# hku-mars/BALM

Hardware: AMD Instinct MI355X
Metric: BA iterations/sec (W poses x F plane features) (higher is better)
Workload: dtype f64

## Files before the change

### balm_amd/capi.py

```python
import ctypes as C
import os

import numpy as np

_HERE = os.path.dirname(os.path.abspath(__file__))
LIB_PATH = os.environ.get("BALM_HIP_LIB") or os.path.join(_HERE, "lib", "libbalm_hip.so")

FORM_LEFT, FORM_RIGHT = 0, 1
OK, ERR_ARG, ERR_HIP, ERR_STATE, ERR_TOO_FEW_PLANES, ERR_NUMERIC = range(6)
ABI_VERSION = 6
FLAG_TIMING = 1
FLAG_LOOPBACK_SHARDS = 2
FLAG_SYRK_INT8 = 4
T_MOMENTS, T_FACTORS, T_SYRK, T_ASSEMBLE, T_SOLVE, T_UPDATE, T_BUILD, T_VOXEL, T_COV, T_COMM, T_UPLOAD, T_COUNT = range(12)
TIMING_NAMES = ["moments", "factors", "syrk", "assemble", "solve", "update", "build", "voxel", "cov", "comm", "upload"]

EXPORTS = ["balm_create", "balm_prewarm", "balm_create_multi", "balm_destroy", "balm_set_features", "balm_set_features_cb", "balm_evaluate", "balm_only_residual",
           "balm_solve_damped", "balm_damping_iter", "balm_build_clusters", "balm_build_clusters_planes", "balm_voxel_defaults", "balm_associate", "balm_associate_scans", "balm_get_features", "balm_get_association", "balm_pose_covariance",
           "balm_window_open", "balm_window_add_scan", "balm_window_add_scan_strided", "balm_window_recut", "balm_window_get_points", "balm_window_features", "balm_window_marginalize", "balm_window_info", "balm_window_close",
           "balm_set_allreduce", "balm_comm_unique_id", "balm_comm_init_rank", "balm_comm_info",
           "balm_get_timing", "balm_get_shard_timing", "balm_get_solve_trace", "balm_chain_macro_plan", "balm_reset_timing", "balm_work_model", "balm_last_error", "balm_version", "balm_abi_version"]


class IterLog(C.Structure):
    _fields_ = [("r1", C.c_double), ("r2", C.c_double), ("u", C.c_double), ("v", C.c_double),
                ("q", C.c_double), ("q1", C.c_double), ("accepted", C.c_int), ("hess_evaluated", C.c_int)]


class LMOpts(C.Structure):
    _fields_ = [("form", C.c_int), ("u0", C.c_double), ("max_iter", C.c_int), ("rel_tol", C.c_double),
                ("min_planes_per_pose", C.c_int), ("force_hess", C.c_int), ("no_stop", C.c_int),
                ("verbose", C.c_int), ("reanchor", C.c_int), ("abs_tol", C.c_double)]


class VoxelOpts(C.Structure):
    _fields_ = [("voxel_size", C.c_double), ("eigen_thr", C.c_float * 3), ("min_ps", C.c_int), ("layer_limit", C.c_int),
                ("min_observers", C.c_int), ("fix_frames", C.c_int), ("max_plane_dist", C.c_double),
                ("max_lambda21", C.c_double), ("max_lambda0", C.c_double), ("want_point_features", C.c_int),
                ("fix_point_limit", C.c_int), ("defer_recut", C.c_int)]


ALLREDUCE_FN = C.CFUNCTYPE(C.c_int, C.c_void_p, C.c_long, C.c_void_p)
FILL_CLUSTERS_FN = C.CFUNCTYPE(None, C.c_void_p, C.c_int, C.c_int, C.POINTER(C.c_double))

_LIB = None


class BalmError(RuntimeError):
    def __init__(self, code, msg):
        super().__init__("balm_hip error %d: %s" % (code, msg))
        self.code = code


def lib():
    global _LIB
    if _LIB is None:
        if not os.path.exists(LIB_PATH):
            raise ImportError("libbalm_hip.so is not built (%s missing): run `python -m balm_amd.build`. "
                              "There is no CPU fallback for the HIP path." % LIB_PATH)
        L = C.CDLL(LIB_PATH)
        abi = getattr(L, "balm_abi_version", None)
        abi = abi() if abi is not None else 0
        if abi != ABI_VERSION:
            raise ImportError("libbalm_hip.so has ABI revision %d, this binding was written for %d: rebuild (python -m balm_amd.build)"
                              % (abi, ABI_VERSION))
        L.balm_create.restype = C.c_void_p
        L.balm_create.argtypes = [C.c_int, C.c_int, C.c_int]
        L.balm_create_multi.restype = C.c_void_p
        L.balm_create_multi.argtypes = [C.c_int, C.c_int, C.c_int, C.c_int]
        L.balm_prewarm.argtypes = [C.c_int]
        L.balm_destroy.restype = None
        L.balm_destroy.argtypes = [C.c_void_p]
        L.balm_set_features.argtypes = [C.c_void_p, C.c_int, C.c_void_p, C.c_void_p, C.c_void_p]
        L.balm_set_features_cb.argtypes = [C.c_void_p, C.c_int, FILL_CLUSTERS_FN, C.c_void_p, C.c_void_p, C.c_void_p]
        L.balm_evaluate.argtypes = [C.c_void_p, C.c_int, C.c_void_p, C.c_int, C.c_int, C.c_void_p, C.c_void_p,
                                    C.POINTER(C.c_double)]
        L.balm_only_residual.argtypes = [C.c_void_p, C.c_void_p, C.POINTER(C.c_double)]
        L.balm_solve_damped.argtypes = [C.c_void_p, C.c_void_p, C.c_void_p, C.c_double, C.c_void_p,
                                        C.POINTER(C.c_double)]
        L.balm_damping_iter.argtypes = [C.c_void_p, C.POINTER(LMOpts), C.c_void_p, C.POINTER(IterLog),
                                        C.POINTER(C.c_int)]
        L.balm_build_clusters.argtypes = [C.c_void_p, C.c_int, C.c_void_p, C.c_void_p, C.c_void_p, C.c_long,
                                          C.c_void_p, C.c_void_p, C.c_void_p]
        L.balm_build_clusters_planes.argtypes = [C.c_void_p, C.c_int, C.c_void_p, C.c_void_p, C.c_size_t, C.c_size_t, C.c_void_p,
                                                 C.c_void_p, C.c_void_p]
        L.balm_associate_scans.argtypes = [C.c_void_p, C.POINTER(VoxelOpts), C.c_int, C.c_void_p, C.c_void_p, C.c_size_t,
                                           C.c_void_p, C.POINTER(C.c_int), C.POINTER(C.c_long)]
        L.balm_window_add_scan_strided.argtypes = [C.c_void_p, C.c_void_p, C.c_long, C.c_size_t, C.c_void_p]
        L.balm_window_open.argtypes = [C.c_void_p, C.POINTER(VoxelOpts)]
        L.balm_window_add_scan.argtypes = [C.c_void_p, C.c_void_p, C.c_long, C.c_void_p]
        L.balm_window_recut.argtypes = [C.c_void_p]
        L.balm_window_get_points.argtypes = [C.c_void_p, C.c_void_p, C.c_void_p, C.c_void_p, C.c_long, C.c_void_p]
        L.balm_window_features.argtypes = [C.c_void_p, C.POINTER(C.c_int)]
        L.balm_window_marginalize.argtypes = [C.c_void_p, C.c_int, C.c_void_p]
        L.balm_window_info.argtypes = [C.c_void_p, C.POINTER(C.c_int), C.POINTER(C.c_long), C.POINTER(C.c_long)]
        L.balm_window_close.argtypes = [C.c_void_p]
        L.balm_associate.argtypes = [C.c_void_p, C.POINTER(VoxelOpts), C.c_void_p, C.c_void_p, C.c_long, C.c_void_p,
                                     C.POINTER(C.c_int), C.POINTER(C.c_long)]
        L.balm_get_features.argtypes = [C.c_void_p, C.c_void_p, C.c_void_p, C.c_void_p]
        L.balm_get_association.argtypes = [C.c_void_p, C.c_void_p, C.c_void_p]
        L.balm_voxel_defaults.restype = None
        L.balm_voxel_defaults.argtypes = [C.POINTER(VoxelOpts)]
        L.balm_pose_covariance.argtypes = [C.c_void_p, C.c_void_p, C.c_void_p, C.c_double, C.c_void_p, C.c_void_p]
        L.balm_set_allreduce.argtypes = [C.c_void_p, ALLREDUCE_FN, C.c_void_p]
        L.balm_comm_unique_id.argtypes = [C.c_void_p]
        L.balm_comm_init_rank.argtypes = [C.c_void_p, C.c_int, C.c_int, C.c_void_p]
        L.balm_comm_info.argtypes = [C.c_void_p, C.c_void_p]
        L.balm_get_timing.argtypes = [C.c_void_p, C.c_void_p, C.c_void_p]
        L.balm_get_shard_timing.argtypes = [C.c_void_p, C.c_int, C.c_void_p, C.c_void_p]
        L.balm_get_solve_trace.argtypes = [C.c_void_p, C.c_void_p, C.c_long, C.c_void_p]
        L.balm_chain_macro_plan.argtypes = [C.c_int, C.c_int, C.c_void_p, C.c_long]
        L.balm_reset_timing.argtypes = [C.c_void_p]
        L.balm_work_model.argtypes = [C.c_void_p, C.c_void_p]
        L.balm_last_error.restype = C.c_char_p
        L.balm_last_error.argtypes = [C.c_void_p]
        L.balm_version.restype = C.c_char_p
        _LIB = L
    return _LIB


def chain_macro_plan(panels, helpers):
    tab = np.empty(helpers * 64, np.int32)
    rc = lib().balm_chain_macro_plan(int(panels), int(helpers), tab.ctypes.data_as(C.c_void_p), tab.size)
    if rc != OK:
        raise BalmError(rc, "balm_chain_macro_plan(%d, %d)" % (panels, helpers))
    tab = tab.reshape(helpers, 64)
    return [[(int(e) & 0xffff, int(e) >> 16) for e in row if e >= 0] for row in tab]


def _p(a):
    return None if a is None else a.ctypes.data_as(C.c_void_p)


def _c(a, dtype=np.float64):
    return None if a is None else np.ascontiguousarray(a, dtype=dtype)


class Context:

    def __init__(self, win_size, device=0, flags=0, n_devices=None):
        self.L = lib()
        self.W = int(win_size)
        self.n = 6 * self.W
        if n_devices is None:
            self.h = self.L.balm_create(self.W, int(device), int(flags))
        else:
            self.h = self.L.balm_create_multi(self.W, int(device), int(n_devices), int(flags))
        if not self.h:
            raise BalmError(ERR_HIP, "balm_create(win_size=%d, device=%d, n_devices=%s) failed (no GPU, bad device, or "
                                     "win_size out of range)" % (win_size, device, n_devices))
        self.F = 0
        self._cb = None

    def close(self):
        if getattr(self, "h", None):
            self.L.balm_destroy(self.h)
            self.h = None

    def __del__(self):
        try:
            self.close()
        except Exception:
            pass

    def _check(self, rc):
        if rc != OK:
            raise BalmError(rc, self.L.balm_last_error(self.h).decode())

    def set_features(self, clusters, fix, coeffs):
        clusters, fix, coeffs = _c(clusters), _c(fix), _c(coeffs)
        F = clusters.shape[0]
        assert clusters.shape == (F, self.W, 10), clusters.shape
        assert coeffs.shape == (F,)
        assert fix is None or fix.shape == (F, 10)
        self._check(self.L.balm_set_features(self.h, F, _p(clusters), _p(fix), _p(coeffs)))
        self.F = F

    def set_features_cb(self, per_feature, fix, coeffs):
        tabs = [_c(t) for t in per_feature]
        F = len(tabs)
        assert all(t.shape == (self.W, 10) for t in tabs)
        fix, coeffs = _c(fix), _c(coeffs)
        row = self.W * 10

        failed = []

        def fill(_user, f0, f1, dst):
            out = np.ctypeslib.as_array(dst, shape=((f1 - f0) * row,))
            try:
                for a in range(f0, f1):
                    out[(a - f0) * row:(a - f0 + 1) * row] = tabs[a].reshape(-1)
            except BaseException as exc:
                out[:] = 0.0
                failed.append(exc)

        cb = FILL_CLUSTERS_FN(fill)
        rc = self.L.balm_set_features_cb(self.h, F, cb, None, _p(fix), _p(coeffs))
        if failed:
            self.F = 0
            raise failed[0]
        self._check(rc)
        self.F = F

    def build_clusters(self, F, xyz, feat_id, pose_id, fix, coeffs, want_clusters=True):
        xyz = _c(xyz, np.float32).reshape(-1, 3)
        feat_id, pose_id = _c(feat_id, np.int32), _c(pose_id, np.int32)
        fix, coeffs = _c(fix), _c(coeffs)
        out = np.zeros((F, self.W, 10)) if want_clusters else None
        self._check(self.L.balm_build_clusters(self.h, F, _p(xyz), _p(feat_id), _p(pose_id), xyz.shape[0],
                                               _p(fix), _p(coeffs), _p(out)))
        self.F = F
        return out

    @staticmethod
    def _containers(arrays):
        keep = [np.ascontiguousarray(a, dtype=np.float32) for a in arrays]
        keep = [a.reshape(-1, 3) if a.ndim == 1 else a for a in keep]
        cols = {a.shape[1] for a in keep}
        assert len(cols) == 1 and min(cols) >= 3, "every container: [n, c] float32 with the same c >= 3"
        ptrs = (C.c_void_p * len(keep))(*[a.ctypes.data if a.shape[0] else None for a in keep])
        cnt = (C.c_long * len(keep))(*[a.shape[0] for a in keep])
        return ptrs, cnt, 4 * cols.pop(), keep

    def build_clusters_planes(self, planes, pose_col, fix, coeffs, want_clusters=True):
        ptrs, cnt, stride, keep = self._containers(planes)
        F = len(keep)
        fix, coeffs = _c(fix), _c(coeffs)
        out = np.zeros((F, self.W, 10)) if want_clusters else None
        self._check(self.L.balm_build_clusters_planes(self.h, F, ptrs, cnt, stride, 4 * int(pose_col), _p(fix), _p(coeffs), _p(out)))
        self.F = F
        return out

    def associate_scans(self, scans, poses, voxel_size=2.0, eigen_thresholds=(1.0 / 16, 1.0 / 16, 1.0 / 9), min_ps=15,
                        want_features=True, layer_limit=2, min_observers=2, fix_frames=0, strict=None, want_points=False):
        ptrs, cnt, stride, keep = self._containers(scans)
        poses = _c(poses)
        assert poses.shape[0] == self.W + fix_frames == len(keep), "one scan and one pose per window slot"
        o = self._voxel_opts(voxel_size, eigen_thresholds, min_ps, layer_limit, min_observers, fix_frames, strict, want_points)
        F, nr = C.c_int(0), C.c_long(0)
        self._check(self.L.balm_associate_scans(self.h, C.byref(o), len(keep), ptrs, cnt, stride, _p(poses), C.byref(F), C.byref(nr)))
        self.F = F.value
        return self.F, nr.value, self._association_result(want_features, fix_frames, want_points, sum(a.shape[0] for a in keep))

    def _voxel_opts(self, voxel_size, eigen_thresholds, min_ps, layer_limit, min_observers, fix_frames, strict, want_points):
        o = VoxelOpts()
        self.L.balm_voxel_defaults(C.byref(o))
        o.voxel_size = voxel_size
        o.eigen_thr = (C.c_float * 3)(*[float(t) for t in eigen_thresholds])
        o.min_ps, o.layer_limit, o.min_observers, o.fix_frames = min_ps, layer_limit, min_observers, fix_frames
        if strict is not None:
            o.max_plane_dist, o.max_lambda21, o.max_lambda0 = strict
        o.want_point_features = int(want_points)
        return o

    def _association_result(self, want_features, fix_frames, want_points, n_pts):
        feats = None
        if want_features and self.F > 0:
            cl, co = np.zeros((self.F, self.W, 10)), np.zeros(self.F)
            layer = np.zeros(self.F, dtype=np.int32)
            self._check(self.L.balm_get_features(self.h, _p(cl), _p(co), _p(layer)))
            feats = (cl, co, layer)
            if fix_frames or want_points:
                fix = np.zeros((self.F, 10))
                pf = np.zeros(n_pts, dtype=np.int32) if want_points else None
                self._check(self.L.balm_get_association(self.h, _p(fix), _p(pf)))
                feats = (cl, co, layer, fix, pf)
        return feats

    def associate(self, xyz, frame_id, poses, voxel_size=2.0, eigen_thresholds=(1.0 / 16, 1.0 / 16, 1.0 / 9),
                  min_ps=15, want_features=True, layer_limit=2, min_observers=2, fix_frames=0, strict=None,
                  want_points=False):
        xyz = _c(xyz, np.float32).reshape(-1, 3)
        frame_id, poses = _c(frame_id, np.int32), _c(poses)
        assert poses.shape[0] == self.W + fix_frames, "poses for the marginalised scans too"
        o = self._voxel_opts(voxel_size, eigen_thresholds, min_ps, layer_limit, min_observers, fix_frames, strict, want_points)
        F, nr = C.c_int(0), C.c_long(0)
        self._check(self.L.balm_associate(self.h, C.byref(o), _p(xyz), _p(frame_id), xyz.shape[0], _p(poses),
                                          C.byref(F), C.byref(nr)))
        self.F = F.value
        return self.F, nr.value, self._association_result(want_features, fix_frames, want_points, xyz.shape[0])
# ... 170 lines not shown
```

### balm_amd/csrc/balm_capi.hip

```cpp
#include <algorithm>
#include <array>
#include <atomic>
#include <chrono>
#include <cmath>
#include <cstdio>
#include <cstdlib>
#include <cstring>

#include "balm_internal.h"

using namespace balm;

#define HIP_TRY(expr)                                                                              \
  do {                                                                                             \
    hipError_t e_ = (expr);                                                                        \
    if (e_ != hipSuccess) {                                                                        \
      ctx->err = std::string(#expr) + ": " + hipGetErrorString(e_);                                \
      return BALM_ERR_HIP;                                                                         \
    }                                                                                              \
  } while (0)

namespace {

#ifdef BALM_COLD_TRACE
// ... 72 lines not shown
void collect_timing(balm_ctx *c) {
  for (auto &sp : c->timer.pending) {
    float ms = 0;
    if (hipEventElapsedTime(&ms, sp.a, sp.b) == hipSuccess) { c->timer.ms[sp.slot] += ms; c->timer.cnt[sp.slot]++; }
    c->timer.pool.push_back(sp.a); c->timer.pool.push_back(sp.b);
  }
  c->timer.pending.clear();
}

template <class T>
int dalloc(balm_ctx *ctx, T **p, size_t count) {
  if (*p) { hipFree(*p); *p = nullptr; }
  if (count == 0) count = 1;
  HIP_TRY(hipMalloc((void **)p, count * sizeof(T)));
  return BALM_OK;
}

template <class T>
int keep(balm_ctx *ctx, T **p, size_t *cap, size_t count) {
  if (*p && *cap >= count) return BALM_OK;
  for (int k = 0; k < balm_ctx::LM_GRAPHS; k++)
    if (ctx->lm_graph[k]) { hipGraphExecDestroy(ctx->lm_graph[k]); ctx->lm_graph[k] = nullptr; ctx->lm_graph_form[k] = -1; }
  int rc = dalloc(ctx, p, count + count / 4);
  *cap = rc ? 0 : count + count / 4;
  return rc;
}

template <class T>
int ensure(balm_ctx *ctx, T **p, size_t *cap, size_t count) {
  if (*p && *cap >= count) return BALM_OK;
  for (int k = 0; k < balm_ctx::LM_GRAPHS; k++)
    if (ctx->lm_graph[k]) { hipGraphExecDestroy(ctx->lm_graph[k]); ctx->lm_graph[k] = nullptr; ctx->lm_graph_form[k] = -1; }
  int rc = dalloc(ctx, p, count);
  if (rc) return rc;
  *cap = count;
  return BALM_OK;
}

int stage_begin(balm_ctx *ctx, size_t total_bytes) {
  total_bytes += 16 * 256;
  ctx->stage_off = 0;
  if (ctx->stage_cap >= total_bytes) return BALM_OK;
  if (ctx->d_stage) { hipStreamSynchronize(ctx->stream); hipFree(ctx->d_stage); ctx->d_stage = nullptr; ctx->stage_cap = 0; }
  const size_t want = total_bytes + total_bytes / 8;
  HIP_TRY(hipMalloc((void **)&ctx->d_stage, want));
  ctx->stage_cap = want;
  return BALM_OK;
}

template <class T>
T *stage_take(balm_ctx *ctx, size_t count) {
  const size_t off = (ctx->stage_off + 255) & ~(size_t)255;
  ctx->stage_off = off + count * sizeof(T);
  return reinterpret_cast<T *>(ctx->d_stage + off);
}

int sync_stream(balm_ctx *ctx) {
  HIP_TRY(hipStreamSynchronize(ctx->stream));
  HIP_TRY(hipGetLastError());
  collect_timing(ctx);
  return BALM_OK;
}

long red_dacc_off(const balm_ctx *c) { return (long)c->ntiles * TILE_ELEMS; }
long red_r_off(const balm_ctx *c) { return red_dacc_off(c) + (long)DACC_MAX * c->W; }

bool has_transport(const balm_ctx *ctx) { return ctx->comm || multi_is_loopback(ctx) || ctx->allreduce; }

int hook_allreduce(balm_ctx *ctx, double *buf, long n) {
  if (ctx->comm) { Span sp(ctx, BALM_T_COMM); return comm_allreduce(ctx, buf, n); }
  if (multi_is_loopback(ctx)) { Span sp(ctx, BALM_T_COMM); return loopback_allreduce(ctx, buf, n); }
  if (!ctx->allreduce) return BALM_OK;
  int rc = sync_stream(ctx);
  if (rc) return rc;
  if (ctx->allreduce((void *)buf, n, ctx->allreduce_user) != 0) {
    ctx->err = "all-reduce hook failed";
    return BALM_ERR_STATE;
  }
  return BALM_OK;
}

int set_damping(balm_ctx *ctx, double u) {
  ctx->u_value = u;
  ctx->u_on_device = false;
  return BALM_OK;
}
int push_damping(balm_ctx *ctx) {
  double *slot = ctx->h_scal + 16 + (ctx->u_ring++ & 63);
  *slot = ctx->u_value;
  HIP_TRY(hipMemcpyAsync(ctx->d_scal + SCAL_U, slot, sizeof(double), hipMemcpyHostToDevice, ctx->stream));
  ctx->u_on_device = true;
  return BALM_OK;
}

static void collect_timing_if_idle(balm_ctx *ctx) {
  if (!ctx->timer.on || ctx->timer.pending.empty()) return;
  if (hipStreamSynchronize(ctx->stream) == hipSuccess) collect_timing(ctx);
}

int wait_scalars(balm_ctx *ctx) {
  volatile double *stamp = ctx->h_scal + SCAL_STAMP;
  const double want = (double)ctx->mail_seq;
  const auto t0 = std::chrono::steady_clock::now();
  for (int spin = 0;; spin++) {
    if (*stamp == want) { std::atomic_thread_fence(std::memory_order_acquire); collect_timing_if_idle(ctx); return BALM_OK; }
    if ((spin & 255) == 255 && std::chrono::steady_clock::now() - t0 > std::chrono::microseconds(300)) break;
  }
  int rc = sync_stream(ctx);
  if (rc) return rc;
  if (*stamp != want) { ctx->err = "balm_damping_iter: the iteration's scalars did not arrive"; return BALM_ERR_HIP; }
  return BALM_OK;
}

void drop_lm_graphs(balm_ctx *ctx) {
  for (int k = 0; k < balm_ctx::LM_GRAPHS; k++) {
    if (ctx->lm_graph[k]) hipGraphExecDestroy(ctx->lm_graph[k]);
    ctx->lm_graph[k] = nullptr; ctx->lm_graph_form[k] = -1;
  }
}

int residual_device(balm_ctx *ctx, const double *d_poses, int f0, int f1, int slot, bool defer_sum = false, bool send_mail = false) {
  if (f1 <= f0) {
    HIP_TRY(hipMemsetAsync(ctx->d_scal + slot, 0, sizeof(double), ctx->stream));
    ctx->nr_tmp = 0;
  } else {
    Span sp(ctx, BALM_T_MOMENTS);
    launch_world_moments(ctx->stream, ctx->d_cl, d_poses, ctx->W, f0, f1, ctx->d_C);
    const EigenMail mail{ctx->d_scal, ctx->d_hscal, send_mail ? (double)++ctx->mail_seq : 0.0, slot};
    ctx->nr_tmp = launch_feature_eigen(ctx->stream, ctx->d_C, ctx->has_fix ? ctx->d_fix : nullptr, ctx->d_coe, f0, f1, ctx->d_feat_tmp,
                                       ctx->d_rpart_tmp, send_mail ? &mail : nullptr);
    if (!defer_sum) launch_sum_scalar(ctx->stream, ctx->d_rpart_tmp, ctx->nr_tmp, ctx->d_scal + slot);
  }
  HIP_TRY(hipGetLastError());
  if (defer_sum) return BALM_OK;
  return hook_allreduce(ctx, ctx->d_scal + slot, 1);
}

bool fuse_trial(const balm_ctx *ctx) {
  const char *e = getenv("BALM_FUSE_TRIAL");
  return ctx->W <= 256 && ctx->F > 0 && e && e[0] == '1';
}

static bool syrk_int8_mode(const balm_ctx *ctx) {
  if (ctx->flags & BALM_FLAG_SYRK_INT8) return true;
  const char *m = getenv("BALM_SYRK");
  return m && !strcmp(m, "int8");
}
static bool syrk_int8_for(const balm_ctx *ctx, long K) {
  if (!syrk_int8_mode(ctx)) return false;
  if (const char *m = getenv("BALM_SYRK_INT8_MIN_COLS")) return K >= atol(m);
  return K >= 12288L && ctx->W >= 96;
}

int prepare_evaluate(balm_ctx *ctx, int form, int nf) {
  if (nf <= 0) return BALM_OK;
  const SyrkPlan plan = plan_syrk(ctx->ntiles, 3L * nf);
  int rc;
  size_t gcols = (size_t)plan.Kpad + 64, parts = (size_t)plan.SG * ctx->ntiles;
  if (ctx->sparse && nf == ctx->F) {
    gcols = (size_t)ctx->sp_nchunks * ctx->sp_nsteps * 4 + 64;
    parts = (size_t)ctx->sp_nitems;
  }
  {
    const double *before = ctx->d_Gt;
    if ((rc = ensure(ctx, &ctx->d_Gt, &ctx->cap_Gt, gcols * ctx->npad))) return rc;
    if (ctx->d_Gt != before) ctx->gt_dirty_cols = ~(size_t)0;
  }
  if ((rc = ensure(ctx, &ctx->d_part, &ctx->cap_part, parts * TILE_ELEMS))) return rc;
  if (syrk_int8_for(ctx, 3L * nf) && !(ctx->sparse && nf == ctx->F)) {
    if ((rc = ensure(ctx, &ctx->d_i8, &ctx->cap_i8, syrk_i8_scratch_bytes(ctx->n, 3L * nf, nullptr)))) return rc;
    if (!ctx->d_rowmax) ctx->rowmax_cur_valid = false;
    if (!ctx->d_rowmax2) ctx->rowmax_trial_valid = false;
    if ((rc = ensure(ctx, &ctx->d_rowmax, &ctx->cap_rowmax, (size_t)ctx->npad + 128))) return rc;
    if ((rc = ensure(ctx, &ctx->d_rowmax2, &ctx->cap_rowmax2, (size_t)ctx->npad + 128))) return rc;
    if ((rc = ensure(ctx, &ctx->d_rowmax_part, &ctx->cap_rowmax_part, (size_t)factors_grid(ctx->W, nf, form) * 6 * ctx->W))) return rc;
    HIP_TRY(prepare_device_syrk_i8());
  }
  if ((rc = ensure(ctx, &ctx->d_dpart, &ctx->cap_dpart, (size_t)factors_grid(ctx->W, nf, form) * DACC_MAX * ctx->W))) return rc;
  if (nf == ctx->F && fuse_trial(ctx)) {
    if (ctx->cap_Gt2 < gcols * ctx->npad || ctx->cap_dpart2 < (size_t)factors_grid(ctx->W, nf, form) * DACC_MAX * ctx->W) ctx->gt_trial_valid = false;
    if ((rc = ensure(ctx, &ctx->d_Gt2, &ctx->cap_Gt2, gcols * ctx->npad))) return rc;
    if ((rc = ensure(ctx, &ctx->d_dpart2, &ctx->cap_dpart2, (size_t)factors_grid(ctx->W, nf, form) * DACC_MAX * ctx->W))) return rc;
  }
  return BALM_OK;
}

int evaluate_device(balm_ctx *ctx, int form, const double *d_poses, int f0, int f1, int slot) {
  const int W = ctx->W, nf = f1 - f0;
  const int dacc = form == 0 ? DACC_LEFT : DACC_RIGHT;
  int rc;
  if (nf <= 0) {
    HIP_TRY(hipMemsetAsync(ctx->d_red, 0, ctx->red_len * sizeof(double), ctx->stream));
    if ((rc = hook_allreduce(ctx, ctx->d_red, (long)ctx->red_len))) return rc;
    Span sp(ctx, BALM_T_ASSEMBLE);
    launch_assemble(ctx->stream, form, ctx->d_red, red_dacc_off(ctx), ctx->d_sub, ctx->ntiles, W, ctx->d_H, ctx->d_g,
                    ctx->d_red + red_r_off(ctx), ctx->d_scal + slot);
    return BALM_OK;
  }
  SyrkPlan plan = plan_syrk(ctx->ntiles, 3L * nf);
  if ((rc = prepare_evaluate(ctx, form, nf))) return rc;
  const int nblk = factors_grid(W, nf, form);
  hipStream_t s = ctx->stream;
  if (!(ctx->feat_cur_valid && f0 == 0 && f1 == ctx->F)) {
    Span sp(ctx, BALM_T_MOMENTS);
    launch_world_moments(s, ctx->d_cl, d_poses, W, f0, f1, ctx->d_C);
    ctx->nr_cur = launch_feature_eigen(s, ctx->d_C, ctx->has_fix ? ctx->d_fix : nullptr, ctx->d_coe, f0, f1, ctx->d_feat, ctx->d_rpart);
    ctx->feat_cur_valid = (f0 == 0 && f1 == ctx->F);
  }
  const int nr = ctx->nr_cur;
  const bool sparse = ctx->sparse && f0 == 0 && f1 == ctx->F;
  const size_t kpad = sparse ? (size_t)ctx->sp_nchunks * ctx->sp_nsteps * 4 : (size_t)plan.Kpad;
  if (!(ctx->gt_cur_valid && ctx->feat_cur_valid && f0 == 0 && f1 == ctx->F)) {
    Span sp(ctx, BALM_T_FACTORS);
    const size_t k0 = (size_t)3 * nf, k1 = kpad + 64;
    if (ctx->gt_dirty_cols == ~(size_t)0) {
      HIP_TRY(hipMemsetAsync(ctx->d_Gt, 0, ctx->cap_Gt * sizeof(double), s));
      ctx->gt_dirty_cols = 0;
    } else if (ctx->gt_dirty_cols > k0) {
      HIP_TRY(hipMemsetAsync(ctx->d_Gt + k0 * ctx->npad, 0, (std::max(ctx->gt_dirty_cols, k1) - k0) * ctx->npad * sizeof(double), s));
    }
    ctx->gt_dirty_cols = k0;
    ctx->rowmax_cur_valid = launch_factors(s, form, ctx->d_cl, d_poses, ctx->d_feat, W, ctx->npad, f0, f1, ctx->d_Gt, ctx->d_dpart, nblk,
                                           sparse ? ctx->d_slot : nullptr, (!sparse && syrk_int8_for(ctx, 3L * nf)) ? ctx->d_rowmax : nullptr, ctx->d_rowmax_part);
    ctx->gt_cur_valid = false;
  }
  HIP_TRY(hipGetLastError());
  const bool int8 = !sparse && syrk_int8_for(ctx, 3L * nf);
  {
    Span sp(ctx, BALM_T_SYRK);
    if (sparse) launch_syrk_sparse(s, ctx->d_Gt, ctx->npad, ctx->d_jobs, ctx->d_items, ctx->d_chunk_ids, ctx->sp_nsteps, ctx->sp_nitems, ctx->d_part);
    else if (int8) {
      if (launch_syrk_i8(s, ctx->d_Gt, ctx->npad, ctx->n, 3L * nf, ctx->d_sub, ctx->ntiles, ctx->d_i8, ctx->d_part,
                         ctx->rowmax_cur_valid ? ctx->d_rowmax : nullptr)) { ctx->err = "INT8 SYRK: unsupported size"; return BALM_ERR_ARG; }
      plan.SG = 1;
    }
    else launch_syrk(s, ctx->d_Gt, ctx->npad, ctx->ntiles, ctx->d_jobs, plan, ctx->d_part);
  }
  {
    Span sp(ctx, BALM_T_ASSEMBLE);
    launch_reduce(s, ctx->d_part, plan.SG, (long)ctx->ntiles * TILE_ELEMS, ctx->d_dpart, nblk, dacc * W,
                  ctx->d_rpart, nr, ctx->d_red, red_dacc_off(ctx), red_r_off(ctx), sparse ? ctx->d_csr : nullptr);
  }
  if ((rc = hook_allreduce(ctx, ctx->d_red, (long)ctx->red_len))) return rc;
  {
    Span sp(ctx, BALM_T_ASSEMBLE);
    launch_assemble(s, form, ctx->d_red, red_dacc_off(ctx), ctx->d_sub, ctx->ntiles, W, ctx->d_H, ctx->d_g, ctx->d_red + red_r_off(ctx),
                    ctx->d_scal + slot);
  }
  return BALM_OK;
}

int trial_device(balm_ctx *ctx, int form, const double *d_poses, int slot) {
  const int W = ctx->W, F = ctx->F;
  hipStream_t s = ctx->stream;
  const SyrkPlan plan = plan_syrk(ctx->ntiles, 3L * F);
  const bool sparse = ctx->sparse;
  const size_t kpad = sparse ? (size_t)ctx->sp_nchunks * ctx->sp_nsteps * 4 : (size_t)plan.Kpad;
  const int nblk = factors_grid(W, F, form);
  {
    Span sp(ctx, BALM_T_FACTORS);
    const size_t k0 = (size_t)3 * F, k1 = kpad + 64;
    HIP_TRY(hipMemsetAsync(ctx->d_Gt2 + k0 * ctx->npad, 0, (k1 - k0) * ctx->npad * sizeof(double), s));
    if (ctx->npad > ctx->n)
      HIP_TRY(hipMemset2DAsync(ctx->d_Gt2 + ctx->n, (size_t)ctx->npad * sizeof(double), 0,
                               (size_t)(ctx->npad - ctx->n) * sizeof(double), k0, s));
    ctx->nr_tmp = launch_moments_factors(s, form, ctx->d_cl, d_poses, ctx->has_fix ? ctx->d_fix : nullptr, ctx->d_coe, W, ctx->npad, F,
                                         ctx->d_Gt2, ctx->d_dpart2, nblk, sparse ? ctx->d_slot : nullptr, ctx->d_feat_tmp, ctx->d_rpart_tmp,
                                         (!sparse && syrk_int8_for(ctx, 3L * F) && ctx->d_rowmax2) ? ctx->d_rowmax2 : nullptr, ctx->d_rowmax_part);
    ctx->rowmax_trial_valid = !sparse && syrk_int8_for(ctx, 3L * F) && ctx->d_rowmax2;
  }
  HIP_TRY(hipGetLastError());
  {
    Span sp(ctx, BALM_T_MOMENTS);
    launch_sum_scalar(s, ctx->d_rpart_tmp, ctx->nr_tmp, ctx->d_scal + slot);
  }
  ctx->gt_trial_valid = true;
  return hook_allreduce(ctx, ctx->d_scal + slot, 1);
}

int read_scalars(balm_ctx *ctx) {
  HIP_TRY(hipMemcpyAsync(ctx->h_scal, ctx->d_scal, 16 * sizeof(double), hipMemcpyDeviceToHost, ctx->stream));
  return sync_stream(ctx);
}

std::vector<unsigned char> obs_of(const double *clusters, int F, int W) {
  std::vector<unsigned char> obs((size_t)F * W);
  parallel_ranges(obs.size(), (size_t)1 << 16, [&](size_t lo, size_t hi) {
    for (size_t t = lo; t < hi; t++) obs[t] = clusters[t * 10 + 9] != 0 ? 1 : 0;
  });
  return obs;
}

int feature_bookkeeping(balm_ctx *ctx, int F, const unsigned char *obs, const double *fix, const double *coeffs) {
  const int W = ctx->W;
  ctx->planes_per_pose.assign(W, 0);
  double S = 0, B = 0;
  int bad_a = F, bad_rc = BALM_OK;
  std::mutex mu;
  parallel_ranges((size_t)F, (size_t)(65536 / W + 1), [&](size_t lo, size_t hi) {
    std::vector<int> ppp((size_t)W, 0);
    double s = 0, b = 0;
    int my_bad = F, my_rc = BALM_OK;
    for (size_t a = lo; a < hi; a++) {
      int na = 0;
      const unsigned char *oa = obs + a * W;
      for (int i = 0; i < W; i++)
        if (oa[i]) { ppp[(size_t)i]++; na++; }
      if (my_rc == BALM_OK) {
        if (na == 0 && !(fix && fix[a * 10 + 9] != 0)) { my_bad = (int)a; my_rc = BALM_ERR_NUMERIC; }
        else if (!(coeffs[a] >= 0) || !std::isfinite(coeffs[a])) { my_bad = (int)a; my_rc = BALM_ERR_ARG; }
      }
      s += na; b += 0.5 * na * (na + 1.0);
    }
    std::lock_guard<std::mutex> lk(mu);
    for (int i = 0; i < W; i++) ctx->planes_per_pose[(size_t)i] += ppp[(size_t)i];
    S += s; B += b;
    if (my_rc != BALM_OK && my_bad < bad_a) { bad_a = my_bad; bad_rc = my_rc; }
  });
  if (bad_rc == BALM_ERR_NUMERIC) {
    ctx->err = "feature " + std::to_string(bad_a) + " has no observation and no fix cluster (zero point count)";
    return BALM_ERR_NUMERIC;
  }
  if (bad_rc == BALM_ERR_ARG) {
    ctx->err = "feature " + std::to_string(bad_a) + " has a negative or non-finite weight";
    return BALM_ERR_ARG;
  }
  ctx->work_S = S; ctx->work_B = B;
  return BALM_OK;
}

}

extern "C" {

const char *balm_version(void) { return "balm_hip 0.6.0 (gfx950)"; }
int balm_abi_version(void) { return BALM_ABI_VERSION; }

const char *balm_last_error(balm_ctx *ctx) { return ctx ? ctx->err.c_str() : "null context"; }

static void one_destroy(balm_ctx *ctx);

balm_ctx *balm_create(int win_size, int device, int flags) {
  if (win_size < 1 || win_size > MAX_W) return nullptr;
  cold_mark("balm_create: enter");
  int ndev = 0;
  if (hipGetDeviceCount(&ndev) != hipSuccess || ndev < 1 || device < 0 || device >= ndev) return nullptr;
  if (hipSetDevice(device) != hipSuccess) return nullptr;
  cold_mark("balm_create: hipGetDeviceCount + hipSetDevice");
  warm_start(device);
  if (prepare_device_accum() != hipSuccess || prepare_device_cov() != hipSuccess) return nullptr;
  cold_mark("balm_create: prepare_device (function attributes -> code objects)");
  balm_ctx *ctx = new balm_ctx();
  ctx->W = win_size;
  ctx->n = 6 * win_size;
  ctx->npad = (ctx->n + TILE - 1) / TILE * TILE;
  ctx->T = ctx->npad / TILE;
  ctx->nA = (ctx->n + NB - 1) / NB * NB;
  ctx->device = device;
  ctx->flags = flags;
  ctx->timer.on = (flags & BALM_FLAG_TIMING) != 0;
  auto fail = [&]() -> balm_ctx * { one_destroy(ctx); return nullptr; };
  std::vector<int> jobs, sub;
  {
    const int T = ctx->T, ngroups = T / 5;
    std::vector<std::array<int, 3>> mixed[4];
    std::vector<std::array<int, 2>> pairs;
    for (int r = 0; r < TM; r++) for (int c = r; c < TM; c++) pairs.push_back({r, c});
    for (int k = 0; k < 15; k++) mixed[1].push_back({0, pairs[k][0], pairs[k][1]});
    for (int k = 0; k < 10; k++) mixed[1].push_back({1, pairs[k][0], pairs[k][1]});
    for (int k = 10; k < 15; k++) mixed[2].push_back({1, pairs[k][0], pairs[k][1]});
    for (int k = 0; k < 15; k++) mixed[2].push_back({2, pairs[k][0], pairs[k][1]});
    for (int k = 0; k < 5; k++) mixed[2].push_back({3, pairs[k][0], pairs[k][1]});
    for (int k = 5; k < 15; k++) mixed[3].push_back({3, pairs[k][0], pairs[k][1]});
    for (int k = 0; k < 15; k++) mixed[3].push_back({4, pairs[k][0], pairs[k][1]});
    auto regular = [&](int I, int J) {
      jobs.insert(jobs.end(), {0, I, J, 0});
      for (int t = 0; t < 25; t++) sub.push_back(((TM * I + t / TM) << 16) | (TM * J + t % TM));
    };
    for (int m = 0; m < T; m++) {
      for (int i = 0; i < m; i++) regular(i, m);
      if (m >= TM * ngroups) regular(m, m);
      else if (m % TM == TM - 1) {
        const int b = m - (TM - 1);
        for (int v = 1; v <= 3; v++) {
          jobs.insert(jobs.end(), {v, b, b, 0});
          for (const auto &e : mixed[v]) sub.push_back(((TM * (b + e[0]) + e[1]) << 16) | (TM * (b + e[0]) + e[2]));
        }
      }
    }
  }
  ctx->ntiles = (int)(jobs.size() / 4);
  ctx->h_jobs = jobs;
  if (hipStreamCreateWithFlags(&ctx->stream, hipStreamNonBlocking) != hipSuccess) return fail();
  cold_mark("balm_create: job tables + stream");
  const int W = ctx->W, n = ctx->n, nA = ctx->nA;
  ctx->red_len = (size_t)ctx->ntiles * TILE_ELEMS + (size_t)DACC_MAX * W + 2;
  if (dalloc(ctx, &ctx->d_poses, (size_t)12 * W) || dalloc(ctx, &ctx->d_poses_tmp, (size_t)12 * W) ||
      dalloc(ctx, &ctx->d_red, ctx->red_len) || dalloc(ctx, &ctx->d_jobs, jobs.size()) || dalloc(ctx, &ctx->d_sub, sub.size()) ||
      dalloc(ctx, &ctx->d_H, (size_t)n * n) || dalloc(ctx, &ctx->d_g, (size_t)n) ||
      dalloc(ctx, &ctx->d_A, (size_t)(2 * nA + NB) * nA) || dalloc(ctx, &ctx->d_Wp, (size_t)2 * NB * (2 * nA + NB)) ||
      dalloc(ctx, &ctx->d_dvec, (size_t)nA) || dalloc(ctx, &ctx->d_z, (size_t)nA) || dalloc(ctx, &ctx->d_x, (size_t)16 * nA) ||
      dalloc(ctx, &ctx->d_perm, (size_t)nA) || dalloc(ctx, &ctx->d_flags, (size_t)2 * (2 * (nA / NB) + 1) * (nA / NB) + (nA / NB) + 8) || dalloc(ctx, &ctx->d_minv, (size_t)2 * (nA / NB) * NB * NB) || dalloc(ctx, &ctx->d_dx, (size_t)n) ||
      dalloc(ctx, &ctx->d_scal, (size_t)16) || dalloc(ctx, &ctx->d_pre, (size_t)W + 2))
    return fail();
  if (hipHostMalloc((void **)&ctx->h_scal, (16 + 64 + 8) * sizeof(double), hipHostMallocMapped | hipHostMallocCoherent) != hipSuccess) return fail();
  if (hipHostGetDevicePointer((void **)&ctx->d_hscal, ctx->h_scal, 0) != hipSuccess) return fail();
  ctx->h_scal[SCAL_STAMP] = 0.0;
  if (hipMemcpy(ctx->d_jobs, jobs.data(), jobs.size() * sizeof(int), hipMemcpyHostToDevice) != hipSuccess ||
      hipMemcpy(ctx->d_sub, sub.data(), sub.size() * sizeof(int), hipMemcpyHostToDevice) != hipSuccess)
    return fail();
  if (getenv("BALM_SOLVE_TRACE")) {
    const size_t cnt = (size_t)(2 * (nA / NB) + 1) * (nA / NB) * 6 + (size_t)(nA / NB) * 6;
    if (hipMalloc((void **)&ctx->d_trace, cnt * sizeof(long long)) != hipSuccess) return fail();
    hipMemset(ctx->d_trace, 0, cnt * sizeof(long long));
  }
  {
    std::vector<int> ident(nA);
    for (int i = 0; i < nA; i++) ident[i] = i;
    if (hipMemcpy(ctx->d_perm, ident.data(), (size_t)nA * sizeof(int), hipMemcpyHostToDevice) != hipSuccess) return fail();
  }
  if (hipMemset(ctx->d_scal, 0, 16 * sizeof(double)) != hipSuccess) return fail();
  if (hipMemset(ctx->d_red, 0, ctx->red_len * sizeof(double)) != hipSuccess) return fail();
  if (hipMemset(ctx->d_minv, 0, (size_t)2 * (nA / NB) * NB * NB * sizeof(double)) != hipSuccess) return fail();
  cold_mark("balm_create: device buffers + small copies");
  context_born(device); ctx->counted_live = true;
  return ctx;
}

static void one_destroy(balm_ctx *ctx) {
  if (!ctx) return;
  if (ctx->counted_live) { context_gone(ctx->device); ctx->counted_live = false; }
  comm_destroy(ctx);
  drop_lm_graphs(ctx);
  hipSetDevice(ctx->device);
  if (ctx->stream) hipStreamSynchronize(ctx->stream);
  if (ctx->window) { window_close(ctx->window); ctx->window = nullptr; }
  void *ptrs[] = {ctx->d_cl, ctx->d_fix, ctx->d_coe, ctx->d_poses, ctx->d_poses_tmp, ctx->d_C, ctx->d_feat,
                  ctx->d_Gt, ctx->d_Gt2, ctx->d_dpart2, ctx->d_part, ctx->d_dpart, ctx->d_rpart, ctx->d_feat_tmp, ctx->d_rpart_tmp, ctx->d_red, ctx->d_jobs, ctx->d_sub, ctx->d_H,
                  ctx->d_g, ctx->d_A, ctx->d_Wp, ctx->d_dvec, ctx->d_z, ctx->d_x, ctx->d_perm, ctx->d_dx, ctx->d_scal, ctx->d_arena, ctx->d_pre, ctx->d_flags, ctx->d_minv, ctx->d_macro_tab, ctx->d_trace, ctx->d_slot, ctx->d_items, ctx->d_csr, ctx->d_chunk_ids, ctx->d_stage, ctx->d_i8, ctx->d_rowmax, ctx->d_rowmax2, ctx->d_rowmax_part};
  for (void *p : ptrs) if (p) hipFree(p);
  if (ctx->h_scal) hipHostFree(ctx->h_scal);
  ctx->ring.release();
  if (ctx->amail.host) hipHostFree((void *)ctx->amail.host);
  if (ctx->amail.scan_state) hipFree(ctx->amail.scan_state);
  for (auto &sp : ctx->timer.pending) { hipEventDestroy(sp.a); hipEventDestroy(sp.b); }
  for (auto e : ctx->timer.pool) hipEventDestroy(e);
  if (ctx->stream) hipStreamDestroy(ctx->stream);
  delete ctx;
}

static int build_sparse_plan(balm_ctx *ctx, int F, const unsigned char *obs) {
  ctx->sparse = false;
  const char *mode = getenv("BALM_SYRK");
  if (mode && !strcmp(mode, "dense")) return BALM_OK;
  if (syrk_int8_for(ctx, 3L * F)) return BALM_OK;
  const int W = ctx->W, T = ctx->T, ntiles = ctx->ntiles;
  if (T > 128 || T <= 2 || F < 64) return BALM_OK;
  struct Key { uint64_t hi, lo; int a; };
  std::vector<Key> keys((size_t)F);
  parallel_ranges((size_t)F, (size_t)(65536 / W + 1), [&](size_t a0, size_t a1) {
    for (size_t a = a0; a < a1; a++) {
      uint64_t hi = 0, lo = 0;
      const unsigned char *oa = obs + a * W;
      for (int i = 0; i < W; i++)
        if (oa[i])
          for (int b = (6 * i) / TILE; b <= (6 * i + 5) / TILE; b++) {
            if (b < 64) hi |= 1ull << (63 - b); else lo |= 1ull << (127 - b);
          }
      keys[a] = {hi, lo, (int)a};
    }
  });
  auto first_of = [&](const Key &k) { for (int b = 0; b < T; b++) if (b < 64 ? (k.hi >> (63 - b)) & 1 : (k.lo >> (127 - b)) & 1) return b; return T; };
  auto last_of = [&](const Key &k) { for (int b = T - 1; b >= 0; b--) if (b < 64 ? (k.hi >> (63 - b)) & 1 : (k.lo >> (127 - b)) & 1) return b; return -1; };
  std::vector<int> fb((size_t)F), lb((size_t)F);
  for (int a = 0; a < F; a++) { fb[(size_t)a] = first_of(keys[(size_t)a]); lb[(size_t)a] = last_of(keys[(size_t)a]); }
  std::sort(keys.begin(), keys.end(), [&](const Key &x, const Key &y) {
    if (fb[(size_t)x.a] != fb[(size_t)y.a]) return fb[(size_t)x.a] < fb[(size_t)y.a];
    if (lb[(size_t)x.a] != lb[(size_t)y.a]) return lb[(size_t)x.a] < lb[(size_t)y.a];
    return x.hi != y.hi ? x.hi > y.hi : (x.lo != y.lo ? x.lo > y.lo : x.a < y.a);
  });
  const int C = 16, nsteps = 3 * C / 4, nchunks = (F + C - 1) / C;
  auto touched = [](const Key &k, int b) { return b < 64 ? (k.hi >> (63 - b)) & 1 : (k.lo >> (127 - b)) & 1; };
  std::vector<int> slot((size_t)F);
  std::vector<std::vector<int>> chunks_of((size_t)ntiles);
  long total = 0;
  for (int c = 0; c < nchunks; c++) {
    Key cm{0, 0, 0};
    for (int k = c * C; k < F && k < (c + 1) * C; k++) { cm.hi |= keys[(size_t)k].hi; cm.lo |= keys[(size_t)k].lo; slot[(size_t)keys[(size_t)k].a] = k; }
    for (int j = 0; j < ntiles; j++) {
      const int type = ctx->h_jobs[(size_t)4 * j], I = ctx->h_jobs[(size_t)4 * j + 1], J = ctx->h_jobs[(size_t)4 * j + 2];
      bool need;
      if (type == 0) need = touched(cm, I) && touched(cm, J);
      else if (type == 1) need = touched(cm, I) || touched(cm, I + 1);
      else if (type == 2) need = touched(cm, I + 1) || touched(cm, I + 2) || touched(cm, I + 3);
      else need = touched(cm, I + 3) || touched(cm, I + 4);
      if (need) { chunks_of[(size_t)j].push_back(c); total++; }
    }
  }
  const double dense_steps = (double)ntiles * ((3.0 * F + 3) / 4), sparse_steps = (double)total * nsteps;
  const bool forced = mode && !strcmp(mode, "sparse");
  if (total == 0 || (!forced && !(sparse_steps < 0.8 * dense_steps))) return BALM_OK;
  long per = total / 2048;
  if (per < 8) per = 8;
  std::vector<int> items, chunk_ids, csr((size_t)ntiles + 1, 0);
  struct Order { int first_chunk, item; };
  std::vector<Order> order;
  int run = 0;
  for (int j = 0; j < ntiles; j++) {
    csr[(size_t)j] = run;
    const std::vector<int> &L = chunks_of[(size_t)j];
    const long pieces = ((long)L.size() + per - 1) / per;
    for (long q = 0; q < pieces; q++) {
      const size_t b = (size_t)((long)L.size() * q / pieces), e = (size_t)((long)L.size() * (q + 1) / pieces);
      order.push_back({L[b], (int)(items.size() / 4)});
      items.insert(items.end(), {j, (int)chunk_ids.size(), (int)(e - b), run++});
      chunk_ids.insert(chunk_ids.end(), L.begin() + (long)b, L.begin() + (long)e);
    }
  }
  csr[(size_t)ntiles] = run;
  std::stable_sort(order.begin(), order.end(), [](const Order &x, const Order &y) { return x.first_chunk < y.first_chunk; });
  std::vector<int> sorted_items;
  sorted_items.reserve(items.size());
  for (const Order &o : order) sorted_items.insert(sorted_items.end(), items.begin() + 4L * o.item, items.begin() + 4L * o.item + 4);
  if (chunk_ids.empty()) chunk_ids.push_back(0);
  int rc;
  if ((rc = keep(ctx, &ctx->d_slot, &ctx->cap_slot, (size_t)F)) || (rc = keep(ctx, &ctx->d_items, &ctx->cap_items, sorted_items.size())) ||
      (rc = keep(ctx, &ctx->d_chunk_ids, &ctx->cap_chunk_ids, chunk_ids.size())) || (rc = keep(ctx, &ctx->d_csr, &ctx->cap_csr, csr.size())))
    return rc;
  HIP_TRY(hipMemcpy(ctx->d_slot, slot.data(), slot.size() * sizeof(int), hipMemcpyHostToDevice));
  HIP_TRY(hipMemcpy(ctx->d_items, sorted_items.data(), sorted_items.size() * sizeof(int), hipMemcpyHostToDevice));
  HIP_TRY(hipMemcpy(ctx->d_chunk_ids, chunk_ids.data(), chunk_ids.size() * sizeof(int), hipMemcpyHostToDevice));
  HIP_TRY(hipMemcpy(ctx->d_csr, csr.data(), csr.size() * sizeof(int), hipMemcpyHostToDevice));
  ctx->sparse = true; ctx->sp_nsteps = nsteps; ctx->sp_nchunks = nchunks; ctx->sp_nitems = run; ctx->sp_steps = sparse_steps;
  return BALM_OK;
}

static int install_feature_buffers(balm_ctx *ctx, int F, const double *fix, const double *coeffs,
                                   hipMemcpyKind kind = hipMemcpyHostToDevice) {
  int rc;
  drop_lm_graphs(ctx);
  ctx->has_fix = fix != nullptr;
  if (fix) {
    if ((rc = keep(ctx, &ctx->d_fix, &ctx->cap_fix, (size_t)F * 10))) return rc;
    HIP_TRY(hipMemcpyAsync(ctx->d_fix, fix, (size_t)F * 10 * sizeof(double), kind, ctx->stream));
  }
  if ((rc = keep(ctx, &ctx->d_coe, &ctx->cap_coe, (size_t)F))) return rc;
  HIP_TRY(hipMemcpyAsync(ctx->d_coe, coeffs, (size_t)F * sizeof(double), kind, ctx->stream));
  if ((rc = keep(ctx, &ctx->d_C, &ctx->cap_C, (size_t)F * 10))) return rc;
  if ((rc = keep(ctx, &ctx->d_feat, &ctx->cap_feat, (size_t)F * FEAT_STRIDE))) return rc;
  if ((rc = keep(ctx, &ctx->d_feat_tmp, &ctx->cap_feat_tmp, (size_t)F * FEAT_STRIDE))) return rc;
  if ((rc = keep(ctx, &ctx->d_rpart, &ctx->cap_rpart, (size_t)(F + 255) / 256 + 1024 + 1))) return rc;
  if ((rc = keep(ctx, &ctx->d_rpart_tmp, &ctx->cap_rpart_tmp, (size_t)(F + 255) / 256 + 1024 + 1))) return rc;
  ctx->feat_cur_valid = false; ctx->gt_cur_valid = false;
  ctx->F = F;
  return BALM_OK;
}

static int assoc_clusters_host(balm_ctx *ctx);

using FillClusters = std::function<void(int, int, double *, unsigned char *)>;

static int one_set_features_fn(balm_ctx *ctx, int F, const FillClusters &fill, const double *fix, const double *coeffs, bool shard_books = false) {
  if (!ctx) return BALM_ERR_ARG;
  if (ctx->multi && F == 0) { ctx->F = 0; ctx->feat_cur_valid = false; ctx->gt_cur_valid = false; ctx->planes_per_pose.clear(); ctx->work_S = ctx->work_B = 0; return BALM_OK; }
  if (F < 1 || !fill || !coeffs) { ctx->err = "balm_set_features: bad argument"; return BALM_ERR_ARG; }
  HIP_TRY(hipSetDevice(ctx->device));
  const int W = ctx->W;
  const size_t count = (size_t)F * W * 10;
  int rc;
  if ((rc = assoc_clusters_host(ctx))) return rc;
  ctx->F = 0;
  adopt_warm_ring(ctx);
  if ((rc = keep(ctx, &ctx->d_cl, &ctx->cap_cl, count))) return rc;
  if ((rc = stage_begin(ctx, count * sizeof(double)))) return rc;
  double *d_aos = stage_take<double>(ctx, count);
  std::vector<unsigned char> obs((size_t)F * W);
  const size_t unit = (size_t)W * 10 * sizeof(double);
  hipError_t e;
  {
    Span sp(ctx, BALM_T_UPLOAD);
    e = staged_upload(ctx->ring, ctx->device, ctx->stream, d_aos, count * sizeof(double), unit, [&](char *dst, size_t off, size_t len) {
      const int f0 = (int)(off / unit), f1 = f0 + (int)(len / unit);
      fill(f0, f1, reinterpret_cast<double *>(dst), obs.data() + (size_t)f0 * W);
    });
  }
  if (e == hipSuccess) launch_transpose_clusters(ctx->stream, d_aos, ctx->d_cl, F, W);
  HIP_TRY(e);
  if ((!ctx->multi || shard_books) && (rc = feature_bookkeeping(ctx, F, obs.data(), fix, coeffs))) { hipStreamSynchronize(ctx->stream); return rc; }
  if ((rc = build_sparse_plan(ctx, F, obs.data()))) { hipStreamSynchronize(ctx->stream); return rc; }
  if ((rc = install_feature_buffers(ctx, F, fix, coeffs))) { hipStreamSynchronize(ctx->stream); return rc; }
  return sync_stream(ctx);
}

static int one_set_features(balm_ctx *ctx, int F, const double *clusters, const double *fix, const double *coeffs) {
  if (ctx && !(ctx->multi && F == 0) && !clusters) { ctx->err = "balm_set_features: bad argument"; return BALM_ERR_ARG; }
  const size_t row = ctx ? (size_t)ctx->W * 10 : 0;
  return one_set_features_fn(ctx, F, [clusters, row](int f0, int f1, double *dst, unsigned char *o) {
    const double *src = clusters + (size_t)f0 * row;
    stream_copy(dst, src, (size_t)(f1 - f0) * row * sizeof(double));
    const size_t cnt = (size_t)(f1 - f0) * (row / 10);
    for (size_t t = 0; t < cnt; t++) o[t] = src[t * 10 + 9] != 0 ? 1 : 0;
  }, fix, coeffs);
}

static int one_build_clusters(balm_ctx *ctx, int F, const float *xyz, const int *feat_id, const int *pose_id, long n_pts,
// ... 251 lines not shown
  if (arc == -3) { ctx->err = "balm_associate: frame_id out of range or non-finite point"; return BALM_ERR_ARG; }
  if (arc) { ctx->err = arc == -2 ? "balm_associate: unsupported size" : "balm_associate: device failure"; return BALM_ERR_HIP; }
  if (n_root_voxels) *n_root_voxels = nroots;
  if (F == 0) return BALM_OK;
  if (rc) return rc;
  *F_out = F;
  return BALM_OK;
}

static int window_rc(balm_ctx *ctx, const char *who, int rc) {
  if (rc == 0) return BALM_OK;
  ctx->err = std::string(who) + (rc == -2 ? ": window full / bad size / scans that no recut has seen" : rc == -3 ? ": non-finite point or beyond 2^20 voxels" : ": device failure");
  if (rc == -1) ctx->window_dead = true;
  return rc == -1 ? BALM_ERR_HIP : BALM_ERR_ARG;
}

static int window_alive(balm_ctx *ctx, const char *who) {
  if (!ctx->window) { ctx->err = std::string(who) + ": no open window"; return BALM_ERR_STATE; }
  if (ctx->window_dead) { ctx->err = std::string(who) + ": an earlier window call failed on the device; re-open the window (balm_window_open)"; return BALM_ERR_STATE; }
  return BALM_OK;
}

static int one_window_open(balm_ctx *ctx, const balm_voxel_opts *opts) {
  if (!ctx) return BALM_ERR_ARG;
  if (!opts || !(opts->voxel_size > 0) || opts->layer_limit < 0 || opts->layer_limit > 2 || opts->min_observers < 0 || opts->fix_frames < 0 ||
      ctx->W + opts->fix_frames > 512 || opts->max_plane_dist < 0 || opts->max_lambda21 < 0 || opts->max_lambda0 < 0 || opts->fix_point_limit < 0) {
    ctx->err = "balm_window_open: bad argument";
    return BALM_ERR_ARG;
  }
  HIP_TRY(hipSetDevice(ctx->device));
  if (ctx->window) { window_close(ctx->window); ctx->window = nullptr; }
  AssocOpts ao{ctx->W, opts->voxel_size, {opts->eigen_thr[0], opts->eigen_thr[1], opts->eigen_thr[2]}, opts->min_ps, opts->layer_limit,
               opts->min_observers, opts->fix_frames, opts->max_plane_dist, opts->max_lambda21, opts->max_lambda0,
               opts->fix_point_limit > 0 ? opts->fix_point_limit : 50, opts->defer_recut != 0};
  ctx->window = window_open(ctx->stream, ao);
  ctx->window_dead = false;
  if (!ctx->window) { ctx->err = "balm_window_open: allocation failed"; return BALM_ERR_HIP; }
  return BALM_OK;
}

static int one_window_add_scan(balm_ctx *ctx, const float *xyz, long n_pts, const double *pose12) {
  if (!ctx) return BALM_ERR_ARG;
  if (int rcw = window_alive(ctx, "balm_window_add_scan")) return rcw;
  if (!xyz || !pose12 || n_pts < 1) { ctx->err = "balm_window_add_scan: bad argument"; return BALM_ERR_ARG; }
  HIP_TRY(hipSetDevice(ctx->device));
  Span sp(ctx, BALM_T_VOXEL);
  return window_rc(ctx, "balm_window_add_scan", window_add_scan(ctx->window, xyz, n_pts, pose12, true));
}

static int one_window_add_scan_strided(balm_ctx *ctx, const void *points, long n_pts, size_t stride, const double *pose12) {
  if (!ctx) return BALM_ERR_ARG;
  if (int rcw = window_alive(ctx, "balm_window_add_scan")) return rcw;
  StridedPoints sp;
  const void *base[1] = {points};
  const long cnt[1] = {n_pts};
  if (!points || !pose12 || n_pts < 1 || !sp.set(1, base, cnt, stride)) { ctx->err = "balm_window_add_scan_strided: bad argument"; return BALM_ERR_ARG; }
  if (stride == 12) return one_window_add_scan(ctx, static_cast<const float *>(points), n_pts, pose12);
  HIP_TRY(hipSetDevice(ctx->device));
  const size_t bytes = (size_t)n_pts * 12;
  if (bytes > PinnedRing::CHUNK) {
    std::vector<float> flat((size_t)n_pts * 3);
    parallel_ranges((size_t)n_pts, (size_t)1 << 15, [&](size_t lo, size_t hi) { sp.gather(reinterpret_cast<char *>(flat.data() + 3 * lo), (long)lo, (long)(hi - lo)); });
    return one_window_add_scan(ctx, flat.data(), n_pts, pose12);
  }
  adopt_warm_ring(ctx);
  HIP_TRY(ctx->ring.init(ctx->device));
  PinnedRing &ring = ctx->ring;
  const int b = ring.pos;
  if (ring.busy[b]) { HIP_TRY(hipEventSynchronize(ring.ev[b])); ring.busy[b] = false; }
  char *dst = ring.buf[b];
  parallel_ranges((size_t)n_pts, (size_t)1 << 15, [&](size_t lo, size_t hi) {
    sp.gather(dst + 12 * lo, (long)lo, (long)(hi - lo));
  });
  Span span(ctx, BALM_T_VOXEL);
  return window_rc(ctx, "balm_window_add_scan", window_add_scan(ctx->window, reinterpret_cast<const float *>(dst), n_pts, pose12, true));
}

static int one_window_recut(balm_ctx *ctx) {
  if (!ctx) return BALM_ERR_ARG;
  if (int rcw = window_alive(ctx, "balm_window_recut")) return rcw;
  HIP_TRY(hipSetDevice(ctx->device));
  Span sp(ctx, BALM_T_VOXEL);
  return window_rc(ctx, "balm_window_recut", window_recut(ctx->window));
}

static int one_window_marginalize(balm_ctx *ctx, int mg, const double *poses) {
  if (!ctx) return BALM_ERR_ARG;
  if (int rcw = window_alive(ctx, "balm_window_marginalize")) return rcw;
  HIP_TRY(hipSetDevice(ctx->device));
  Span sp(ctx, BALM_T_VOXEL);
  return window_rc(ctx, "balm_window_marginalize", window_marginalize(ctx->window, mg, poses));
}

static int one_window_features(balm_ctx *ctx, int *F_out) {
  if (!ctx) return BALM_ERR_ARG;
  if (int rcw = window_alive(ctx, "balm_window_features")) return rcw;
  if (!F_out) { ctx->err = "balm_window_features: bad argument"; return BALM_ERR_ARG; }
  HIP_TRY(hipSetDevice(ctx->device));
  *F_out = 0;
  ctx->F = 0;
  ctx->assoc_clusters.clear(); ctx->assoc_coeffs.clear(); ctx->assoc_layer.clear(); ctx->assoc_fix.clear(); ctx->assoc_point_feat.clear(); ctx->assoc_cl_on_device = false;
  int F = 0, *d_lay = nullptr;
  double *d_out = nullptr, *d_coe = nullptr, *d_fix = nullptr;
  int rc;
  {
    Span sp(ctx, BALM_T_VOXEL);
    rc = window_features(ctx->window, window_min_observers(ctx->window), &F, &d_out, &d_coe, &d_fix, &d_lay);
  }
  if (rc) return window_rc(ctx, "balm_window_features", rc);
  if (F == 0) return BALM_OK;
  if ((rc = install_associated(ctx, F, d_out, d_coe, d_fix, d_lay, nullptr, 0, true, false))) return rc;
  *F_out = F;
  return BALM_OK;
}

int balm_get_features(balm_ctx *ctx, double *clusters, double *coeffs, int *layer) {
  if (!ctx) return BALM_ERR_ARG;
  if (ctx->assoc_coeffs.empty()) { ctx->err = "balm_get_features: no balm_associate result"; return BALM_ERR_STATE; }
  if (clusters) {
    if (int rc = assoc_clusters_host(ctx)) return rc;
    if (ctx->assoc_clusters.empty()) { ctx->err = "balm_get_features: the association's table is gone"; return BALM_ERR_STATE; }
    std::memcpy(clusters, ctx->assoc_clusters.data(), ctx->assoc_clusters.size() * sizeof(double));
  }
  if (coeffs) std::memcpy(coeffs, ctx->assoc_coeffs.data(), ctx->assoc_coeffs.size() * sizeof(double));
  if (layer) std::memcpy(layer, ctx->assoc_layer.data(), ctx->assoc_layer.size() * sizeof(int));
  return BALM_OK;
}

int balm_get_association(balm_ctx *ctx, double *fix, int *point_feature) {
  if (!ctx) return BALM_ERR_ARG;
  if (ctx->assoc_coeffs.empty()) { ctx->err = "balm_get_association: no balm_associate result"; return BALM_ERR_STATE; }
  if (point_feature && ctx->assoc_point_feat.empty()) {
    ctx->err = "balm_get_association: want_point_features was not set"; return BALM_ERR_STATE;
  }
  if (fix) std::memcpy(fix, ctx->assoc_fix.data(), ctx->assoc_fix.size() * sizeof(double));
  if (point_feature) std::memcpy(point_feature, ctx->assoc_point_feat.data(), ctx->assoc_point_feat.size() * sizeof(int));
  return BALM_OK;
}

static int one_pose_covariance(balm_ctx *ctx, const double *poses, const double *cluster_cov, double point_sigma, double *Rcov,
                         double *Rcov_raw) {
  if (!ctx) return BALM_ERR_ARG;
  if (!ctx->multi && ctx->F < 1) { ctx->err = "balm_pose_covariance: no features installed"; return BALM_ERR_STATE; }
  if (!poses || (!cluster_cov && !(point_sigma > 0))) { ctx->err = "balm_pose_covariance: bad argument"; return BALM_ERR_ARG; }
  if (ctx->W > MAX_W_LDS) { ctx->err = "balm_pose_covariance: windows above 480 poses are not supported"; return BALM_ERR_ARG; }
  HIP_TRY(hipSetDevice(ctx->device));
  const int W = ctx->W, n = ctx->n, nA = ctx->nA, F = ctx->F;
  hipStream_t s = ctx->stream;
  HIP_TRY(hipMemcpyAsync(ctx->d_poses, poses, (size_t)12 * W * sizeof(double), hipMemcpyHostToDevice, s));
  ctx->feat_cur_valid = false; ctx->gt_cur_valid = false;
  int rc = evaluate_device(ctx, BALM_FORM_LEFT, ctx->d_poses, 0, F, 0);
  ctx->feat_cur_valid = false; ctx->gt_cur_valid = false;
  if (rc) return rc;
  const SyrkPlan plan = plan_syrk(ctx->ntiles, 3L * (F > 0 ? F : 1));
  const size_t gcols = (size_t)plan.Kpad + 64, tiles = (size_t)ctx->ntiles * TILE_ELEMS;
  if ((rc = ensure(ctx, &ctx->d_Gt, &ctx->cap_Gt, 2 * gcols * ctx->npad))) return rc;
  ctx->gt_dirty_cols = ~(size_t)0;
  if ((rc = ensure(ctx, &ctx->d_part, &ctx->cap_part, (size_t)plan.SG * tiles))) return rc;
  const int nblk = cov_factors_grid(W, F > 0 ? F : 1);
  if ((rc = ensure(ctx, &ctx->d_dpart, &ctx->cap_dpart, (size_t)nblk * DACC_MAX * W))) return rc;
  const bool int8 = F > 0 && syrk_int8_for(ctx, 3L * F);
  if (int8) {
    if ((rc = ensure(ctx, &ctx->d_i8, &ctx->cap_i8, syrk_i8_scratch_bytes(ctx->n, 3L * F, nullptr)))) return rc;
    HIP_TRY(prepare_device_syrk_i8());
  }
  const size_t pay = 2 * tiles + (size_t)21 * W, nn = (size_t)n * n;
  const size_t ncc = (cluster_cov && F > 0) ? (size_t)F * W * 81 : 0;
  if ((rc = stage_begin(ctx, (pay + 2 * nn + 2 * (size_t)nA * nA + ncc) * sizeof(double)))) return rc;
  double *buf = stage_take<double>(ctx, pay + 2 * nn + 2 * (size_t)nA * nA), *d_cc = nullptr;
  double *redx = buf, *redy = buf + tiles, *sdiag = buf + 2 * tiles, *Rraw = buf + pay, *Rc = Rraw + nn,
         *T0 = Rc + nn, *T1 = T0 + (size_t)nA * nA;
  hipError_t e = hipSuccess;
  if (ncc) {
    d_cc = stage_take<double>(ctx, ncc);
    adopt_warm_ring(ctx);
    if (e == hipSuccess) { Span sp(ctx, BALM_T_UPLOAD); e = staged_copy(ctx->ring, ctx->device, s, d_cc, cluster_cov, (size_t)F * W * 81 * sizeof(double)); }
  }
  double *Gx = ctx->d_Gt, *Gy = ctx->d_Gt + gcols * ctx->npad;
  if (e == hipSuccess && F == 0) e = hipMemsetAsync(buf, 0, pay * sizeof(double), s);
  if (e == hipSuccess && F > 0) {
    Span sp(ctx, BALM_T_COV);
    const size_t k0 = (size_t)3 * F;
    hipMemsetAsync(Gx + k0 * ctx->npad, 0, (gcols - k0) * ctx->npad * sizeof(double), s);
    hipMemsetAsync(Gy + k0 * ctx->npad, 0, (gcols - k0) * ctx->npad * sizeof(double), s);
    launch_cov_factors(s, ctx->d_cl, d_cc, point_sigma * point_sigma, ctx->d_poses, ctx->d_feat, W, ctx->npad, F, Gx, Gy,
                       ctx->d_dpart, nblk);
    e = hipGetLastError();
    if (int8) {
      if (launch_syrk_i8(s, Gx, ctx->npad, ctx->n, 3L * F, ctx->d_sub, ctx->ntiles, ctx->d_i8, ctx->d_part)) e = hipErrorInvalidValue;
      launch_cov_reduce_tiles(s, ctx->d_part, 1, (long)tiles, redx);
      if (launch_syrk_i8(s, Gy, ctx->npad, ctx->n, 3L * F, ctx->d_sub, ctx->ntiles, ctx->d_i8, ctx->d_part)) e = hipErrorInvalidValue;
      launch_cov_reduce_tiles(s, ctx->d_part, 1, (long)tiles, redy);
    } else {
      launch_syrk(s, Gx, ctx->npad, ctx->ntiles, ctx->d_jobs, plan, ctx->d_part);
      launch_cov_reduce_tiles(s, ctx->d_part, plan.SG, (long)tiles, redx);
      launch_syrk(s, Gy, ctx->npad, ctx->ntiles, ctx->d_jobs, plan, ctx->d_part);
      launch_cov_reduce_tiles(s, ctx->d_part, plan.SG, (long)tiles, redy);
    }
    launch_cov_reduce_dacc(s, ctx->d_dpart, nblk, W, sdiag);
  }
  if (e == hipSuccess) rc = hook_allreduce(ctx, buf, (long)pay);
  if (e == hipSuccess && !rc) {
    Span sp(ctx, BALM_T_COV);
    launch_cov_assemble(s, redx, redy, sdiag, ctx->d_sub, ctx->ntiles, W, Rraw);
    hipMemsetAsync(ctx->d_g, 0, (size_t)n * sizeof(double), s);
    set_damping(ctx, 0.0);
    ctx->need_minv = true;
    launch_solve(ctx, true);
    ctx->need_minv = false;
    launch_congruence_inverse(ctx, Rraw, T0, T1, Rc);
    if (Rcov) e = hipMemcpyAsync(Rcov, Rc, nn * sizeof(double), hipMemcpyDeviceToHost, s);
    if (e == hipSuccess && Rcov_raw) e = hipMemcpyAsync(Rcov_raw, Rraw, nn * sizeof(double), hipMemcpyDeviceToHost, s);
  }
  if (e == hipSuccess) e = hipStreamSynchronize(s);
  if (e == hipSuccess) e = hipGetLastError();
  if (rc) return rc;
  HIP_TRY(e);
  collect_timing(ctx);
  return BALM_OK;
}

int balm_comm_info(balm_ctx *ctx, long *out4) {
  if (!ctx || !out4) return BALM_ERR_ARG;
  out4[0] = 1; out4[1] = 0; out4[2] = (long)ctx->red_len; out4[3] = 0;
  if (ctx->comm) {
    int cnt = -1, rk = -1;
    comm_query(ctx, &cnt, &rk);
    out4[0] = cnt; out4[1] = rk; out4[3] = 1;
  } else if (multi_is_loopback(ctx)) {
    out4[0] = ctx->multi->n; out4[1] = ctx->rank; out4[3] = 2;
  } else if (ctx->allreduce) {
    out4[0] = -1; out4[3] = 3;
  }
  return BALM_OK;
}

int balm_set_allreduce(balm_ctx *ctx, balm_allreduce_fn fn, void *user) {
  if (!ctx) return BALM_ERR_ARG;
  if (fn && (ctx->multi || ctx->comm)) { ctx->err = "balm_set_allreduce: the context already has a collective transport"; return BALM_ERR_STATE; }
  ctx->allreduce = fn;
  ctx->allreduce_user = user;
  return BALM_OK;
}

static int one_evaluate(balm_ctx *ctx, int form, const double *poses, int head, int end, double *Hess, double *JacT,
                  double *residual) {
  if (!ctx) return BALM_ERR_ARG;
  if (!ctx->multi) {
    if (ctx->F < 1) { ctx->err = "balm_evaluate: no features installed"; return BALM_ERR_STATE; }
    if ((form != 0 && form != 1) || !poses || head < 0 || end > ctx->F || head >= end) {
      ctx->err = "balm_evaluate: bad argument"; return BALM_ERR_ARG;
    }
  }
  HIP_TRY(hipSetDevice(ctx->device));
  const int n = ctx->n;
  HIP_TRY(hipMemcpyAsync(ctx->d_poses, poses, (size_t)12 * ctx->W * sizeof(double), hipMemcpyHostToDevice, ctx->stream));
  ctx->feat_cur_valid = false; ctx->gt_cur_valid = false;
  int rc = evaluate_device(ctx, form, ctx->d_poses, head, end, 0);
  ctx->feat_cur_valid = false; ctx->gt_cur_valid = false;
  if (rc) return rc;
  if (Hess) HIP_TRY(hipMemcpyAsync(Hess, ctx->d_H, (size_t)n * n * sizeof(double), hipMemcpyDeviceToHost, ctx->stream));
  if (JacT) HIP_TRY(hipMemcpyAsync(JacT, ctx->d_g, (size_t)n * sizeof(double), hipMemcpyDeviceToHost, ctx->stream));
  if ((rc = read_scalars(ctx))) return rc;
  if (residual) *residual = ctx->h_scal[0];
  if (!std::isfinite(ctx->h_scal[0])) { ctx->err = "balm_evaluate: non-finite residual"; return BALM_ERR_NUMERIC; }
  return BALM_OK;
}

static int one_only_residual(balm_ctx *ctx, const double *poses, double *residual) {
  if (!ctx) return BALM_ERR_ARG;
  if (!ctx->multi && ctx->F < 1) { ctx->err = "balm_only_residual: no features installed"; return BALM_ERR_STATE; }
  if (!poses || !residual) { ctx->err = "balm_only_residual: bad argument"; return BALM_ERR_ARG; }
  HIP_TRY(hipSetDevice(ctx->device));
  HIP_TRY(hipMemcpyAsync(ctx->d_poses_tmp, poses, (size_t)12 * ctx->W * sizeof(double), hipMemcpyHostToDevice, ctx->stream));
  int rc = residual_device(ctx, ctx->d_poses_tmp, 0, ctx->F, 1);
  if (rc) return rc;
  if ((rc = read_scalars(ctx))) return rc;
  *residual = ctx->h_scal[1];
  if (!std::isfinite(ctx->h_scal[1])) { ctx->err = "balm_only_residual: non-finite residual"; return BALM_ERR_NUMERIC; }
  return BALM_OK;
}

int balm_solve_damped(balm_ctx *ctx, const double *Hess, const double *JacT, double u, double *dxi, double *q1) {
  if (!ctx) return BALM_ERR_ARG;
  if (!Hess || !JacT || !dxi) { ctx->err = "balm_solve_damped: bad argument"; return BALM_ERR_ARG; }
  HIP_TRY(hipSetDevice(ctx->device));
  const int n = ctx->n;
  HIP_TRY(hipMemcpyAsync(ctx->d_H, Hess, (size_t)n * n * sizeof(double), hipMemcpyHostToDevice, ctx->stream));
  HIP_TRY(hipMemcpyAsync(ctx->d_g, JacT, (size_t)n * sizeof(double), hipMemcpyHostToDevice, ctx->stream));
  {
    Span sp(ctx, BALM_T_SOLVE);
    int rcu = set_damping(ctx, u);
    if (rcu) return rcu;
    launch_solve(ctx, true);
  }
  HIP_TRY(hipMemcpyAsync(dxi, ctx->d_dx, (size_t)n * sizeof(double), hipMemcpyDeviceToHost, ctx->stream));
  int rc = read_scalars(ctx);
  if (rc) return rc;
  if (!std::isfinite(ctx->h_scal[2]) && !ctx->persistent_off && solve_timed_out(ctx)) {
    ctx->persistent_off = true;
    {
      Span sp(ctx, BALM_T_SOLVE);
      launch_solve(ctx, true);
    }
    HIP_TRY(hipMemcpyAsync(dxi, ctx->d_dx, (size_t)n * sizeof(double), hipMemcpyDeviceToHost, ctx->stream));
    if ((rc = read_scalars(ctx))) return rc;
  }
  if (q1) *q1 = ctx->h_scal[2];
  return BALM_OK;
}

static int lm_enqueue(balm_ctx *ctx, int form, bool evaluated, bool mail) {
  int rc;
  if (evaluated && (rc = evaluate_device(ctx, form, ctx->d_poses, 0, ctx->F, 0))) return rc;
  {
    Span sp(ctx, BALM_T_SOLVE);
    launch_solve(ctx, evaluated, form, ctx->d_poses, ctx->d_poses_tmp);
  }
  ctx->gt_trial_valid = false;
  bool sum_in_mail = false;
  if (fuse_trial(ctx) && ctx->d_Gt2 && ctx->d_dpart2) {
    if ((rc = trial_device(ctx, form, ctx->d_poses_tmp, 1))) return rc;
  } else {
    sum_in_mail = mail && !has_transport(ctx) && ctx->F > 0;
    const bool eigen_mails = sum_in_mail && ctx->F <= 256;
    if ((rc = residual_device(ctx, ctx->d_poses_tmp, 0, ctx->F, 1, sum_in_mail, eigen_mails))) return rc;
    if (eigen_mails) return BALM_OK;
  }
  if (mail) launch_scalars_mail(ctx->stream, ctx->d_scal, ctx->d_hscal, (double)++ctx->mail_seq, sum_in_mail ? ctx->d_rpart_tmp : nullptr,
                                ctx->nr_tmp, 1);
  else HIP_TRY(hipMemcpyAsync(ctx->h_scal, ctx->d_scal, 16 * sizeof(double), hipMemcpyDeviceToHost, ctx->stream));
  return BALM_OK;
}

static int lm_iteration(balm_ctx *ctx, int form, bool evaluated, int it) {
  const char *genv = getenv("BALM_GRAPH");
  const bool disabled = !(genv && (!strcmp(genv, "1") || !strcmp(genv, "debug")));
  const bool graphable = !disabled && ctx->graphs_ok && it >= 1 && !ctx->timer.on && !has_transport(ctx) && !ctx->multi &&
                         ctx->feat_cur_valid && ctx->F > 0 && !solve_is_persistent(ctx);
  if (graphable) {
    const bool fused = fuse_trial(ctx) && ctx->d_Gt2 && ctx->d_dpart2;
    const int slot = (ctx->gt_parity ? 16 : 0) | (fused ? 8 : 0) | (ctx->gt_cur_valid ? 4 : 0) | (evaluated ? 2 : 0) | ctx->parity;
    if (ctx->lm_graph[slot] && ctx->lm_graph_form[slot] != form) {
      hipGraphExecDestroy(ctx->lm_graph[slot]); ctx->lm_graph[slot] = nullptr;
    }
    if (!ctx->lm_graph[slot]) {
      hipGraph_t g = nullptr;
      ctx->u_on_device = true;
      bool ok = hipStreamBeginCapture(ctx->stream, hipStreamCaptureModeThreadLocal) == hipSuccess;
      if (ok) {
// ... 382 lines not shown
  for (int a = 0; a < F; a++) cum[(size_t)a + 1] = cum[(size_t)a] + (double)plane_count[a] + 1.0;
  multi_cut(m, F, cum);
  const size_t Wc = (size_t)ctx->W;
  int rc = multi_run(m, [&](int k) {
    const int f0 = m->fbeg[(size_t)k], nf = m->fbeg[(size_t)k + 1] - f0;
    if (nf == 0) return one_set_features(m->sub[(size_t)k], 0, nullptr, nullptr, nullptr);
    StridedPoints part;
    if (!part.set(nf, plane_points + f0, plane_count + f0, stride_bytes, pose_offset_bytes)) return (int)BALM_ERR_ARG;
    return one_build_clusters(m->sub[(size_t)k], nf, nullptr, nullptr, nullptr, 0, fix ? fix + (size_t)f0 * 10 : nullptr, coeffs + f0,
                              clusters_out ? clusters_out + (size_t)f0 * Wc * 10 : nullptr, &part);
  });
  return multi_done(ctx, m, F, rc, "balm_build_clusters_planes");
}

int balm_window_add_scan_strided(balm_ctx *ctx, const void *points, long n_pts, size_t stride_bytes, const double *pose12) {
  return one_window_add_scan_strided(ctx, points, n_pts, stride_bytes, pose12);
}

int balm_window_open(balm_ctx *ctx, const balm_voxel_opts *opts) { return one_window_open(ctx, opts); }
int balm_window_add_scan(balm_ctx *ctx, const float *xyz, long n_pts, const double *pose12) {
  return one_window_add_scan(ctx, xyz, n_pts, pose12);
}
int balm_window_recut(balm_ctx *ctx) { return one_window_recut(ctx); }
int balm_window_marginalize(balm_ctx *ctx, int mg_size, const double *poses) { return one_window_marginalize(ctx, mg_size, poses); }
int balm_window_features(balm_ctx *ctx, int *F_out) {
  balm_multi *m = leader_of(ctx);
  if (!m) return one_window_features(ctx, F_out);
  ctx->multi = nullptr;
  int rc = one_window_features(ctx, F_out);
  ctx->multi = m;
  m->F = 0;
  if (rc || *F_out == 0) return rc;
  if ((rc = assoc_clusters_host(ctx))) return rc;
  return multi_set_features(ctx, m, *F_out, ctx->assoc_clusters.data(), ctx->assoc_fix.data(), ctx->assoc_coeffs.data());
}
int balm_window_info(balm_ctx *ctx, int *scans, long *points, long *nodes) {
  if (!ctx) return BALM_ERR_ARG;
  if (!ctx->window) { ctx->err = "balm_window_info: no open window"; return BALM_ERR_STATE; }
  if (scans) *scans = window_count(ctx->window);
  if (points) *points = window_points(ctx->window);
  if (nodes) *nodes = window_nodes(ctx->window);
  return BALM_OK;
}
int balm_window_get_points(balm_ctx *ctx, float *xyz, int *slot, int *feature, long capacity, long *n_out) {
  if (!ctx) return BALM_ERR_ARG;
  if (int rcw = window_alive(ctx, "balm_window_get_points")) return rcw;
  if (!n_out || capacity < 0) { ctx->err = "balm_window_get_points: bad argument"; return BALM_ERR_ARG; }
  HIP_TRY(hipSetDevice(ctx->device));
  const long n = window_get_points(ctx->window, xyz, slot, feature, capacity);
  if (n == -2) { ctx->err = "balm_window_get_points: capacity too small"; return BALM_ERR_ARG; }
  if (n < 0) return window_rc(ctx, "balm_window_get_points", -1);
  *n_out = n;
  return BALM_OK;
}
int balm_window_close(balm_ctx *ctx) {
  if (!ctx) return BALM_ERR_ARG;
  if (ctx->window) { hipSetDevice(ctx->device); window_close(ctx->window); ctx->window = nullptr; }
  return BALM_OK;
}

int balm_evaluate(balm_ctx *ctx, int form, const double *poses, int head, int end, double *Hess, double *JacT, double *residual) {
  balm_multi *m = leader_of(ctx);
  if (!m) return one_evaluate(ctx, form, poses, head, end, Hess, JacT, residual);
  if (m->F < 1) { ctx->err = "balm_evaluate: no features installed"; return BALM_ERR_STATE; }
  if ((form != 0 && form != 1) || !poses || head < 0 || end > m->F || head >= end) { ctx->err = "balm_evaluate: bad argument"; return BALM_ERR_ARG; }
  return multi_run(m, [&](int k) {
    const int f0 = m->fbeg[(size_t)k], f1 = m->fbeg[(size_t)k + 1];
    const int lh = (head > f0 ? head : f0) - f0, le = (end < f1 ? end : f1) - f0;
    double r = 0;
    return one_evaluate(m->sub[(size_t)k], form, poses, lh, le > lh ? le : lh, k ? nullptr : Hess, k ? nullptr : JacT, k ? &r : residual);
  });
}

int balm_only_residual(balm_ctx *ctx, const double *poses, double *residual) {
  balm_multi *m = leader_of(ctx);
  if (!m) return one_only_residual(ctx, poses, residual);
  if (m->F < 1) { ctx->err = "balm_only_residual: no features installed"; return BALM_ERR_STATE; }
  if (!poses || !residual) { ctx->err = "balm_only_residual: bad argument"; return BALM_ERR_ARG; }
  return multi_run(m, [&](int k) { double r = 0; return one_only_residual(m->sub[(size_t)k], poses, k ? &r : residual); });
}

int balm_damping_iter(balm_ctx *ctx, const balm_lm_opts *o, double *poses, balm_iter_log *log, int *n_iters) {
  balm_multi *m = leader_of(ctx);
  if (!m) return one_damping_iter(ctx, o, poses, log, n_iters);
  if (m->F < 1) { ctx->err = "balm_damping_iter: no features installed"; return BALM_ERR_STATE; }
  if (!o || !poses || o->max_iter < 1) { ctx->err = "balm_damping_iter: bad argument"; return BALM_ERR_ARG; }
  const size_t np = (size_t)12 * ctx->W;
  std::vector<std::vector<double>> pk((size_t)m->n, std::vector<double>(poses, poses + np));
  std::vector<int> its((size_t)m->n, 0);
  balm_lm_opts ok = *o;
  int rc = multi_run(m, [&](int k) {
    balm_lm_opts oo = ok;
    if (k) oo.verbose = 0;
    return one_damping_iter(m->sub[(size_t)k], &oo, pk[(size_t)k].data(), k ? nullptr : log, &its[(size_t)k]);
  });
  if (rc) { if (ctx->err.empty()) for (auto *q : m->sub) if (!q->err.empty()) { ctx->err = q->err; break; } return rc; }
  std::memcpy(poses, pk[0].data(), np * sizeof(double));
  if (n_iters) *n_iters = its[0];
  return BALM_OK;
}

int balm_pose_covariance(balm_ctx *ctx, const double *poses, const double *cluster_cov, double point_sigma, double *Rcov,
                         double *Rcov_raw) {
  balm_multi *m = leader_of(ctx);
  if (!m) return one_pose_covariance(ctx, poses, cluster_cov, point_sigma, Rcov, Rcov_raw);
  if (m->F < 1) { ctx->err = "balm_pose_covariance: no features installed"; return BALM_ERR_STATE; }
  const size_t W = (size_t)ctx->W;
  return multi_run(m, [&](int k) {
    const size_t f0 = (size_t)m->fbeg[(size_t)k];
    return one_pose_covariance(m->sub[(size_t)k], poses, cluster_cov ? cluster_cov + f0 * W * 81 : nullptr, point_sigma,
                               k ? nullptr : Rcov, k ? nullptr : Rcov_raw);
  });
}

int balm_get_solve_trace(balm_ctx *ctx, long long *ticks, long capacity, int *dims3) {
  if (!ctx || !dims3) return BALM_ERR_ARG;
  const int P = ctx->nA / NB, RB = 2 * P + 1;
  dims3[0] = RB; dims3[1] = P; dims3[2] = 6;
  if (!ctx->d_trace) { ctx->err = "balm_get_solve_trace: create the context with BALM_SOLVE_TRACE=1 in the environment"; return BALM_ERR_STATE; }
  if (!ticks || capacity < (long)RB * P * 6 + 6L * P) { ctx->err = "balm_get_solve_trace: buffer too small"; return BALM_ERR_ARG; }
  HIP_TRY(hipSetDevice(ctx->device));
  HIP_TRY(hipStreamSynchronize(ctx->stream));
  HIP_TRY(hipMemcpy(ticks, ctx->d_trace, ((size_t)RB * P * 6 + 6 * (size_t)P) * sizeof(long long), hipMemcpyDeviceToHost));
  return BALM_OK;
}

int balm_get_timing(balm_ctx *ctx, double *ms, long *count) {
  if (!ctx) return BALM_ERR_ARG;
  for (int k = 0; k < BALM_T_COUNT; k++) {
    if (ms) ms[k] = ctx->timer.ms[k];
    if (count) count[k] = ctx->timer.cnt[k];
  }
  return BALM_OK;
}

int balm_get_shard_timing(balm_ctx *ctx, int shard, double *ms, long *count) {
  if (!ctx) return BALM_ERR_ARG;
  balm_ctx *q = ctx;
  if (ctx->multi) {
    if (shard < 0 || shard >= ctx->multi->n) { ctx->err = "balm_get_shard_timing: no such shard"; return BALM_ERR_ARG; }
    q = ctx->multi->sub[(size_t)shard];
  } else if (shard != 0) { ctx->err = "balm_get_shard_timing: no such shard"; return BALM_ERR_ARG; }
  return balm_get_timing(q, ms, count);
}

int balm_chain_macro_plan(int panels, int helpers, int *table, long capacity) {
  if (!table || panels < 3 || helpers < 1 || capacity < (long)helpers * 64) return BALM_ERR_ARG;
  std::vector<int> tab;
  if (!balm::chain_macro_plan(panels, helpers, tab)) return BALM_ERR_ARG;
  memcpy(table, tab.data(), tab.size() * sizeof(int));
  return BALM_OK;
}

int balm_reset_timing(balm_ctx *ctx) {
  if (!ctx) return BALM_ERR_ARG;
  for (int k = 0; k < BALM_T_COUNT; k++) { ctx->timer.ms[k] = 0; ctx->timer.cnt[k] = 0; }
  if (balm_multi *m = leader_of(ctx))
    for (size_t q = 1; q < m->sub.size(); q++)
      for (int k = 0; k < BALM_T_COUNT; k++) { m->sub[q]->timer.ms[k] = 0; m->sub[q]->timer.cnt[k] = 0; }
  return BALM_OK;
}

int balm_work_model(balm_ctx *ctx, double *out4) {
  if (!ctx || !out4) return BALM_ERR_ARG;
  const double W = ctx->W, F = ctx->multi ? ctx->multi->F : ctx->F;
  out4[0] = ctx->work_S;
  out4[1] = ctx->work_B;
  if (ctx->multi && ctx->multi->books_per_shard) {
    out4[0] = out4[1] = 0;
    for (const balm_ctx *q : ctx->multi->sub) { out4[0] += q->work_S; out4[1] += q->work_B; }
  }
  (void)W;
  out4[2] = 216.0 * out4[1];
  SyrkPlan p = plan_syrk(ctx->ntiles, 3L * (long)F);
  out4[3] = (double)ctx->ntiles * 25.0 * 2048.0 * ((double)p.Kpad / 4.0);
  if (ctx->sparse && !ctx->multi) out4[3] = ctx->sp_steps * 25.0 * 2048.0;
  if (ctx->multi) {
    double issued = 0;
    for (size_t k = 0; k < ctx->multi->sub.size(); k++) {
      const balm_ctx *q = ctx->multi->sub[k];
      if (q->F < 1) continue;
      if (q->sparse) issued += q->sp_steps * 25.0 * 2048.0;
      else { const SyrkPlan pk = plan_syrk(q->ntiles, 3L * q->F); issued += (double)q->ntiles * 25.0 * 2048.0 * ((double)pk.Kpad / 4.0); }
    }
    out4[3] = issued;
  }
  return BALM_OK;
}

}
```

### balm_amd/csrc/balm_internal.h

```cpp
#pragma once
#include <hip/hip_runtime.h>
#include <atomic>
#include <condition_variable>
#include <cstddef>
#include <cstdint>
#include <functional>
#include <mutex>
#include <string>
#include <thread>
#include <vector>

#include "../../include/balm_hip.h"
#include "host_stage.h"

namespace balm {

constexpr int TILE = 80;
constexpr int TM = 5;
constexpr int TILE_ELEMS = TILE * TILE;
constexpr int FEAT_STRIDE = 24;
constexpr int DACC_LEFT = 27;
constexpr int DACC_RIGHT = 30;
constexpr int DACC_MAX = 30;
constexpr int NB = 48;
constexpr int MAX_W_LDS = 480;
constexpr int MAX_W = 1024;
constexpr int MAX_SHARDS = 16;

enum { FT_NN = 0, FT_VBAR = 1, FT_LAM = 4, FT_U0 = 7, FT_U1 = 10, FT_U2 = 13, FT_C0 = 16, FT_C1 = 17,
       FT_C2 = 18, FT_COE = 19 };

struct Timer {
  bool on = false;
  struct Span { hipEvent_t a, b; int slot; };
  std::vector<Span> pending;
  std::vector<hipEvent_t> pool;
  double ms[BALM_T_COUNT] = {0};
  long cnt[BALM_T_COUNT] = {0};
};

}

namespace balm {
struct WindowSession;
struct AssocMail {
  volatile unsigned int *host = nullptr; unsigned int *dev = nullptr; unsigned int seq = 0;
  unsigned long long *scan_state = nullptr; unsigned int scan_gen = 0;
};
constexpr long SCAN_TILES_CAP = 8192;
}

struct balm_ctx {
  int W = 0, n = 0, npad = 0, T = 0, ntiles = 0, device = 0, flags = 0;
  int nA = 0;
  int F = 0;
  hipStream_t stream = nullptr;
  std::string err;

  double *d_cl = nullptr;
  double *d_fix = nullptr;
  double *d_coe = nullptr;
  double *d_poses = nullptr;
  double *d_poses_tmp = nullptr;
  double *d_C = nullptr;
  double *d_feat = nullptr;
  double *d_feat_tmp = nullptr;
  double *d_rpart_tmp = nullptr;
  int nr_cur = 0, nr_tmp = 0;
  bool feat_cur_valid = false;
  double *d_Gt = nullptr;
  double *d_Gt2 = nullptr, *d_dpart2 = nullptr;
  size_t cap_Gt2 = 0, cap_dpart2 = 0;
  size_t gt_dirty_cols = ~(size_t)0;
  bool gt_cur_valid = false;
  int gt_parity = 0;
  bool gt_trial_valid = false;
  size_t cap_cl = 0, cap_fix = 0, cap_coe = 0, cap_C = 0, cap_feat = 0, cap_feat_tmp = 0, cap_rpart = 0, cap_rpart_tmp = 0;
  size_t cap_slot = 0, cap_items = 0, cap_chunk_ids = 0, cap_csr = 0;
  bool has_fix = false;
  size_t cap_Gt = 0;
  double *d_part = nullptr;
  size_t cap_part = 0;
  double *d_dpart = nullptr;
  size_t cap_dpart = 0;
  double *d_rpart = nullptr;
  double *d_red = nullptr;
  size_t red_len = 0;
  std::vector<int> h_jobs;
  bool sparse = false;
  int sp_nsteps = 0, sp_nchunks = 0, sp_nitems = 0;
  int *d_slot = nullptr;
  int *d_items = nullptr;
  int *d_chunk_ids = nullptr;
  double sp_steps = 0;
  int *d_csr = nullptr;
  int *d_jobs = nullptr;
  int *d_sub = nullptr;
  double *d_H = nullptr;
  double *d_g = nullptr;
  double *d_A = nullptr;
  double *d_Wp = nullptr;
  double *d_dvec = nullptr;
  double *d_z = nullptr;
  double *d_x = nullptr;
  int *d_perm = nullptr;
  int *d_flags = nullptr;
  long long *d_trace = nullptr;
  int fused_cap = -1;
  int chain_cap = -1;
  double *d_minv = nullptr;
  int *d_macro_tab = nullptr;
  int macro_tab_P = 0, macro_tab_NH = 0;
  double *d_dx = nullptr;
  double *d_scal = nullptr;
  double *h_scal = nullptr;
  double *d_hscal = nullptr;
  unsigned long long mail_seq = 0;
  bool need_minv = false;
  bool solve_tiled = false;
  int chain_refused_P[2] = {-1, -1};
  bool solve_backsub = false;
  bool counted_live = false;
  bool persistent_off = false;
  bool inject_solve_timeout = false;
  bool small_ready = false, small_refused = false;
  double u_value = 0.0;
  bool u_on_device = false;
  int u_ring = 0;
  static constexpr int LM_GRAPHS = 32;
  hipGraphExec_t lm_graph[LM_GRAPHS] = {};
  int lm_graph_form[LM_GRAPHS] = {};
  bool graphs_ok = true;
  int parity = 0;
  std::vector<int> planes_per_pose;
  double work_S = 0, work_B = 0;
  std::vector<double> assoc_clusters, assoc_coeffs;
  bool assoc_cl_on_device = false;
  std::vector<int> assoc_layer, assoc_point_feat;
  std::vector<double> assoc_fix;
  balm::WindowSession *window = nullptr;
  bool window_dead = false;
  balm::AssocMail amail;
  void *d_arena = nullptr;
  size_t arena_cap = 0;
  char *d_stage = nullptr;
  size_t stage_cap = 0, stage_off = 0;
  balm::PinnedRing ring;
  balm_allreduce_fn allreduce = nullptr;
  void *allreduce_user = nullptr;
  balm::Timer timer;
  void *comm = nullptr;
  std::atomic<bool> comm_dead{false};
  bool comm_aborted = false;
  std::timed_mutex comm_mu;
  int rank = 0, nranks = 1;
  unsigned long long *d_rowmax = nullptr, *d_rowmax2 = nullptr; size_t cap_rowmax = 0, cap_rowmax2 = 0;
  double *d_rowmax_part = nullptr; size_t cap_rowmax_part = 0;
  bool rowmax_cur_valid = false, rowmax_trial_valid = false;
  unsigned char *d_i8 = nullptr; size_t cap_i8 = 0;
  struct balm_multi *multi = nullptr;
  double *d_pre = nullptr;
};

namespace balm {

hipError_t prepare_device_accum();
hipError_t prepare_device_cov();
hipError_t preload_solve();
hipError_t preload_build();
hipError_t preload_voxel();
void launch_transpose_clusters(hipStream_t s, const double *aos, double *soa, int F, int W);
void launch_world_moments(hipStream_t s, const double *cl, const double *poses, int W, int f0, int f1, double *C);
struct EigenMail { double *scal; double *host; double stamp; int slot; };
int launch_feature_eigen(hipStream_t s, const double *C, const double *fix, const double *coe, int f0, int f1,
                         double *feat, double *rpart, const EigenMail *mail = nullptr);
int factors_grid(int W, int nfeat, int form);
int factors_chunk(int W);
bool launch_factors(hipStream_t s, int form, const double *cl, const double *poses, const double *feat, int W,
                    int npad, int f0, int f1, double *Gt, double *dpart, int nblk, const int *slot = nullptr,
                    unsigned long long *rowmax = nullptr, double *rowmax_part = nullptr);
int launch_moments_factors(hipStream_t s, int form, const double *cl, const double *poses, const double *fix, const double *coe, int W,
                           int npad, int F, double *Gt, double *dpart, int nblk, const int *slot, double *feat, double *rpart,
                           unsigned long long *rowmax = nullptr, double *rowmax_part = nullptr);
struct SyrkPlan { int SG; int nsteps; int Kpad; long nblocks; };
SyrkPlan plan_syrk(int ntiles, long K);
void launch_syrk(hipStream_t s, const double *Gt, int npad, int ntiles, const int *tileIJ, const SyrkPlan &p,
                 double *part);
void launch_syrk_sparse(hipStream_t s, const double *Gt, int npad, const int *jobs, const int *items, const int *chunk_ids,
                        int nsteps, long nitems, double *part);
void launch_reduce(hipStream_t s, const double *part, int SG, long tile_elems_total, const double *dpart, int nblk,
                   int dacc_len, const double *rpart, int nr, double *red, long red_dacc_off, long red_r_off,
                   const int *csr_ptr = nullptr);
void launch_assemble(hipStream_t s, int form, const double *red, long red_dacc_off, const int *tileIJ, int ntiles,
                     int W, double *H, double *g, const double *r_in = nullptr, double *r_out = nullptr);
void launch_sum_scalar(hipStream_t s, const double *rpart, int nr, double *out);
struct I8Layout { int T, rows_p, NT, M; long Kp; size_t off_digits, off_rowmax, off_scale, off_part; };
size_t syrk_i8_scratch_bytes(int n, long K, I8Layout *lay);
hipError_t prepare_device_syrk_i8();
int launch_syrk_i8(hipStream_t s, const double *Gt, int npad, int n, long K, const int *tileIJ, int ntiles, unsigned char *scratch, double *part,
                   const unsigned long long *rowmax_known = nullptr);

struct Barrier;
}

struct balm_multi {
  int n = 0;
  bool loopback = false;
  std::vector<balm_ctx *> sub;
  std::vector<int> fbeg;
  int F = 0;
  bool books_per_shard = false;
  std::vector<std::thread> th;
  std::mutex mu;
  std::condition_variable cv_go, cv_done;
  uint64_t gen = 0;
  int pending = 0;
  bool quit = false;
  const std::function<int(int)> *job = nullptr;
  std::vector<int> rc;
  balm::Barrier *bar = nullptr;
  std::atomic<int> abort_rc{0};
  std::atomic<bool> dead{false};
  std::atomic<uint64_t> lm_seq{0};
  uint64_t lm_epoch = 0;
  double lm_vals[2][8] = {{0}};
  std::vector<hipEvent_t> ev1, ev2;
  std::vector<double *> lb_tmp, lb_buf;
  std::vector<size_t> lb_cap;
};

namespace balm {
balm_multi *multi_new(const std::vector<balm_ctx *> &subs, bool loopback, std::string *err);
void multi_delete(balm_multi *m);
int multi_run(balm_multi *m, const std::function<int(int)> &f);
int comm_unique_id(void *out128);
int comm_init_rank(balm_ctx *ctx, int nranks, int rank, const void *id128);
void comm_destroy(balm_ctx *ctx);
const char *rccl_load_error();
int comm_allreduce(balm_ctx *ctx, double *buf, long n);
void comm_query(const balm_ctx *ctx, int *count, int *rank);
int loopback_allreduce(balm_ctx *ctx, double *buf, long n);
bool multi_is_loopback(const balm_ctx *ctx);
int multi_share_scalars(balm_ctx *ctx, int it, double *vals, int count);
void multi_abort(balm_multi *m, int rc);
int multi_host_barrier_rc(balm_ctx *ctx, int rc);

constexpr int SCAL_U = 5;
constexpr int SCAL_STAMP = 16 + 64;
bool chain_macro_plan(int P, int NH, std::vector<int> &tab);
void context_born(int device);
void context_gone(int device);
bool solve_timed_out(balm_ctx *c);
bool solve_is_persistent(const balm_ctx *c);
void launch_solve(balm_ctx *c, bool new_hessian, int upd_form = 0, const double *upd_poses = nullptr, double *upd_out = nullptr);
void launch_update_poses(hipStream_t s, int form, int W, const double *poses, const double *dx, double *out);
void launch_scalars_mail(hipStream_t s, double *d_scal, double *d_hscal, double stamp, const double *rpart = nullptr, int nr = 0,
                         int slot = 0);
void launch_reanchor(hipStream_t s, int W, double *poses);

struct AssocOpts {
  int W;
  double voxel_size;
  float thr[3];
  int min_ps, layer_limit, min_observers, fix_frames;
  double max_dis, ratio21_max, lam0_max;
  int fix_limit = 50;
  int defer_recut = 0;
};
int associate_device(hipStream_t s, const float *d_xyz, const int *d_frame, const long *d_first, const double *d_poses, long n, const AssocOpts &o,
                     void *arena, size_t arena_cap, size_t *arena_need, int *F_out, double **d_out, double **d_coe,
                     double **d_fix, int **d_layer, int **d_point_feat, long *n_roots, AssocMail *mail, bool *outputs_owned);

WindowSession *window_open(hipStream_t s, const AssocOpts &o);
void window_close(WindowSession *w);
int window_add_scan(WindowSession *w, const float *xyz_new, long n_new, const double *pose12, bool xyz_on_host);
int window_recut(WindowSession *w);
int window_marginalize(WindowSession *w, int mg, const double *poses);
int window_features(WindowSession *w, int min_observers, int *F_out, double **d_out, double **d_coe, double **d_fix, int **d_layer);
long window_get_points(WindowSession *w, float *xyz, int *slot, int *feature, long cap);
int window_count(const WindowSession *w);
int window_min_observers(const WindowSession *w);
long window_points(const WindowSession *w);
long window_nodes(const WindowSession *w);

int cov_factors_grid(int W, int F);
void launch_cov_factors(hipStream_t s, const double *cl, const double *ccov, double sigma2, const double *poses,
                        const double *feat, int W, int npad, int F, double *Gx, double *Gy, double *dpart, int nblk);
void launch_cov_reduce_tiles(hipStream_t s, const double *part, int SG, long tile_total, double *red);
void launch_cov_reduce_dacc(hipStream_t s, const double *dpart, int nblk, int W, double *out);
void launch_cov_assemble(hipStream_t s, const double *redx, const double *redy, const double *sdiag, const int *tileIJ,
                         int ntiles, int W, double *Rout);
void launch_congruence_inverse(balm_ctx *c, const double *Rraw, double *T0, double *T1, double *Rcov);

void launch_build_clusters(hipStream_t s, const float *xyz, const int *feat_id, const int *pose_id, long n_pts,
                           int F, int W, double *soa, int *unsorted_flag);
void launch_build_clusters_any(hipStream_t s, const float *xyz, const int *feat_id, const int *pose_id, long n_pts,
                               int F, int W, double *soa);
void launch_soa_to_aos(hipStream_t s, const double *soa, double *aos, int F, int W);
void launch_rebase_ids(hipStream_t s, int *d_id, long n, int base);
void launch_expand_ids(hipStream_t s, const long *d_first, int m, long n, int *d_id);
void launch_unpack_xyzw(hipStream_t s, const float *d_rec, long n, float *d_xyz, int *d_aux);
void launch_obs_mask(hipStream_t s, const double *soa, int F, int W, unsigned char *mask);

}
```

### balm_amd/csrc/kernels_accum.hip

```cpp
#include "balm_internal.h"

namespace balm {

typedef double d4 __attribute__((ext_vector_type(4)));
typedef double d2 __attribute__((ext_vector_type(2)));

__device__ __forceinline__ double wave_sum(double v) {
#pragma unroll
  for (int off = 32; off > 0; off >>= 1) v += __shfl_xor(v, off, 64);
  return v;
}

struct Obs {
  double N;
  double Rv[3];
  double b[3];
  double Pw[6];
};

__device__ __forceinline__ void to_world(const double P[6], const double v[3], double N, const double R[9],
                                         const double p[3], Obs &o) {
  o.N = N;
#pragma unroll
  for (int r = 0; r < 3; r++) o.Rv[r] = R[r] * v[0] + R[3 + r] * v[1] + R[6 + r] * v[2];
// ... 743 lines not shown

int factors_grid(int W, int nfeat, int form) {
  size_t lds = factors_lds(W, form) + (factors_staged(W, nfeat, form) ? FACTORS_STAGE_BYTES : 0);
  int per_cu = (int)(160 * 1024 / lds);
  if (per_cu < 1) per_cu = 1;
  if (per_cu > 4) per_cu = 4;
  int grid = 256 * per_cu;
  if (grid > nfeat) grid = nfeat;
  if (grid < 1) grid = 1;
  return grid;
}

hipError_t prepare_device_accum() {
  hipError_t e = hipFuncSetAttribute((const void *)k_world_moments, hipFuncAttributeMaxDynamicSharedMemorySize, 160 * 1024);
  if (e == hipSuccess) e = hipFuncSetAttribute((const void *)k_feature_factors<0, false>, hipFuncAttributeMaxDynamicSharedMemorySize, 160 * 1024);
  if (e == hipSuccess) e = hipFuncSetAttribute((const void *)k_feature_factors<1, false>, hipFuncAttributeMaxDynamicSharedMemorySize, 160 * 1024);
  if (e == hipSuccess) e = hipFuncSetAttribute((const void *)k_feature_factors<0, true>, hipFuncAttributeMaxDynamicSharedMemorySize, 160 * 1024);
  if (e == hipSuccess) e = hipFuncSetAttribute((const void *)k_feature_factors<0, true, true>, hipFuncAttributeMaxDynamicSharedMemorySize, 160 * 1024);
  if (e == hipSuccess) e = hipFuncSetAttribute((const void *)k_moments_factors<0, false>, hipFuncAttributeMaxDynamicSharedMemorySize, 160 * 1024);
  if (e == hipSuccess) e = hipFuncSetAttribute((const void *)k_moments_factors<1, false>, hipFuncAttributeMaxDynamicSharedMemorySize, 160 * 1024);
  if (e == hipSuccess) e = hipFuncSetAttribute((const void *)k_moments_factors<0, true>, hipFuncAttributeMaxDynamicSharedMemorySize, 160 * 1024);
  if (e == hipSuccess) e = hipFuncSetAttribute((const void *)k_moments_factors<1, true>, hipFuncAttributeMaxDynamicSharedMemorySize, 160 * 1024);
  return e;
}

int launch_moments_factors(hipStream_t s, int form, const double *cl, const double *poses, const double *fix, const double *coe, int W,
                           int npad, int F, double *Gt, double *dpart, int nblk, const int *slot, double *feat, double *rpart,
                           unsigned long long *rowmax, double *rowmax_part) {
  const int dacc = form == 0 ? DACC_LEFT : DACC_RIGHT;
  const size_t lds = (size_t)((12 + dacc) * W + 80 + 2 * FEAT_STRIDE) * sizeof(double);
  const int bs = (W <= 64 ? 64 : (W <= 128 ? 128 : 256)) + 64;
  if (rowmax) {
    if (form == 0)
      hipLaunchKernelGGL((k_moments_factors<0, true>), dim3(nblk), dim3(bs), lds, s, cl, poses, fix, coe, W, npad, F, Gt, dpart, slot, feat, rpart, rowmax_part);
    else
      hipLaunchKernelGGL((k_moments_factors<1, true>), dim3(nblk), dim3(bs), lds, s, cl, poses, fix, coe, W, npad, F, Gt, dpart, slot, feat, rpart, rowmax_part);
    hipLaunchKernelGGL(k_rowmax_reduce, dim3((npad + 63) / 64), dim3(1024), 0, s, rowmax_part, nblk, W, npad, rowmax);
    return nblk;
  }
  if (form == 0)
    hipLaunchKernelGGL((k_moments_factors<0, false>), dim3(nblk), dim3(bs), lds, s, cl, poses, fix, coe, W, npad, F, Gt, dpart, slot, feat, rpart, nullptr);
  else
    hipLaunchKernelGGL((k_moments_factors<1, false>), dim3(nblk), dim3(bs), lds, s, cl, poses, fix, coe, W, npad, F, Gt, dpart, slot, feat, rpart, nullptr);
  return nblk;
}

bool launch_factors(hipStream_t s, int form, const double *cl, const double *poses, const double *feat, int W,
                    int npad, int f0, int f1, double *Gt, double *dpart, int nblk, const int *slot, unsigned long long *rowmax, double *rowmax_part) {
  const int Wc = factors_chunk(W), chunks = (W + Wc - 1) / Wc;
  size_t lds = factors_lds(W, form);
  int bs = W <= 64 ? 64 : (W <= 128 ? 128 : 256);
  const int staged = factors_staged(W, f1 - f0, form);
  if (staged) lds += FACTORS_STAGE_BYTES;
  const char *er = getenv("BALM_FACTORS_REGS");
  const bool regs = form == 0 && chunks == 1 && W <= bs && !(er && er[0] == '0');
  if (rowmax && regs) {
    hipLaunchKernelGGL((k_feature_factors<0, true, true>), dim3(nblk, chunks), dim3(bs), lds, s, cl, poses, feat, W, Wc, npad, f0, f1, Gt, dpart, slot, staged, rowmax_part);
    hipLaunchKernelGGL(k_rowmax_reduce, dim3((npad + 63) / 64), dim3(1024), 0, s, rowmax_part, nblk, W, npad, rowmax);
    return true;
  }
#define BALM_FACTORS(F, R) hipLaunchKernelGGL((k_feature_factors<F, R, false>), dim3(nblk, chunks), dim3(bs), lds, s, cl, poses, feat, W, Wc, npad, f0, f1, Gt, dpart, slot, staged, nullptr)
  if (form == 0) { if (regs) BALM_FACTORS(0, true); else BALM_FACTORS(0, false); }
  else BALM_FACTORS(1, false);
#undef BALM_FACTORS
  return false;
}

#include "syrk_mfma_asm.inc"

__device__ __forceinline__ void load5(const double *__restrict__ p, double (&x)[TM]) {
#pragma unroll
  for (int r = 0; r < TM; r++) x[r] = p[16 * r];
}

constexpr int SYRK_NBUF = 4;

__device__ __forceinline__ void syrk_sweep(const double *__restrict__ pa, const double *__restrict__ pb, size_t step,
                                           int nsteps) {
  double a[SYRK_NBUF][TM], b[SYRK_NBUF][TM];
#pragma unroll
  for (int i = 0; i < SYRK_NBUF - 1; i++) {
    load5(pa + i * step, a[i]);
    load5(pb + i * step, b[i]);
  }
  pa += (SYRK_NBUF - 1) * step;
  pb += (SYRK_NBUF - 1) * step;
  for (int s = 0; s < nsteps; s += SYRK_NBUF) {
#pragma unroll
    for (int j = 0; j < SYRK_NBUF; j++) {
      const int nb = (j + SYRK_NBUF - 1) % SYRK_NBUF;
      load5(pa, a[nb]);
      load5(pb, b[nb]);
      pa += step; pb += step;
      BALM_SYRK_MFMA_FULL(a[j], b[j])
    }
  }
}

#define BALM_DEFINE_MIXED_SWEEP(V)                                                                                  \
  __device__ __forceinline__ void syrk_sweep_mixed##V(const double *__restrict__ p, size_t step, int nsteps) {    \
    double x[SYRK_NBUF][BALM_SYRK_MIX##V##_NLOAD];                                                                  \
    _Pragma("unroll") for (int i = 0; i < SYRK_NBUF - 1; i++) {                                                    \
      const double *q = p + i * step;                                                                               \
      BALM_SYRK_MIX##V##_LOAD(q, x[i])                                                                              \
    }                                                                                                               \
    p += (SYRK_NBUF - 1) * step;                                                                                    \
    for (int s = 0; s < nsteps; s += SYRK_NBUF) {                                                                   \
      _Pragma("unroll") for (int j = 0; j < SYRK_NBUF; j++) {                                                      \
        const int nb = (j + SYRK_NBUF - 1) % SYRK_NBUF;                                                             \
        BALM_SYRK_MIX##V##_LOAD(p, x[nb])                                                                           \
        p += step;                                                                                                  \
        BALM_SYRK_MIX##V##_MFMA(x[j])                                                                               \
      }                                                                                                             \
    }                                                                                                               \
  }
BALM_DEFINE_MIXED_SWEEP(1)
BALM_DEFINE_MIXED_SWEEP(2)
BALM_DEFINE_MIXED_SWEEP(3)
#undef BALM_DEFINE_MIXED_SWEEP

__device__ __forceinline__ void syrk_accumulate(const double *__restrict__ Gt, int npad, int type, int I, int J,
                                                size_t k_begin, int nsteps) {
  const int lane = threadIdx.x;
  const double *base = Gt + (k_begin + (lane >> 4)) * (size_t)npad + (lane & 15);
  const double *pa = base + I * TILE;
  const double *pb = base + J * TILE;
  const size_t step = (size_t)4 * npad;
  if (type == 0) syrk_sweep(pa, pb, step, nsteps);
  else if (type == 1) syrk_sweep_mixed1(pa, step, nsteps);
  else if (type == 2) syrk_sweep_mixed2(pa, step, nsteps);
  else syrk_sweep_mixed3(pa, step, nsteps);
}

__device__ __forceinline__ void syrk_write_out(double *__restrict__ out) {
  asm volatile("s_nop 15\n\ts_nop 15\n\ts_nop 15" ::: "memory");
  out += threadIdx.x;
#define BALM_X(T)                                                                             \
  {                                                                                           \
    unsigned U[8];                                                                            \
    BALM_SYRK_READ_##T(U);                                                                    \
    _Pragma("unroll") for (int e = 0; e < 4; e++) out[(T * 4 + e) * 64] = __hiloint2double(U[2 * e + 1], U[2 * e]); \
  }
  BALM_SYRK_FOR_TILES(BALM_X)
#undef BALM_X
}

__device__ __forceinline__ long xcd_remap(long bid, long nblocks) {
  const long q = nblocks >> 3, r = nblocks & 7, x = bid & 7;
  return x * q + (x < r ? x : r) + (bid >> 3);
}

__global__ __launch_bounds__(64) void k_hessian_syrk(const double *__restrict__ Gt, int npad, int njobs,
                                                     const int *__restrict__ jobs, int nsteps, long nblocks,
                                                     double *__restrict__ part) {
  const long bid = xcd_remap(blockIdx.x, nblocks);
  const int tile = (int)(bid % njobs);
  const int sg = (int)(bid / njobs);
  BALM_SYRK_ZERO_ACC();
  syrk_accumulate(Gt, npad, jobs[4 * tile], jobs[4 * tile + 1], jobs[4 * tile + 2], (size_t)sg * nsteps * 4, nsteps);
  syrk_write_out(part + ((size_t)sg * njobs + tile) * TILE_ELEMS);
}

__global__ __launch_bounds__(64) void k_hessian_syrk_sparse(const double *__restrict__ Gt, int npad,
                                                            const int *__restrict__ jobs, const int *__restrict__ items,
                                                            const int *__restrict__ chunk_ids, int nsteps, long nitems,
                                                            double *__restrict__ part) {
  const long bid = xcd_remap(blockIdx.x, nitems);
  const int tile = items[4 * bid], first = items[4 * bid + 1], count = items[4 * bid + 2], slot = items[4 * bid + 3];
  const int type = jobs[4 * tile], I = jobs[4 * tile + 1], J = jobs[4 * tile + 2];
  BALM_SYRK_ZERO_ACC();
  for (int c = 0; c < count; c++)
    syrk_accumulate(Gt, npad, type, I, J, (size_t)chunk_ids[first + c] * nsteps * 4, nsteps);
  syrk_write_out(part + (size_t)slot * TILE_ELEMS);
}

SyrkPlan plan_syrk(int ntiles, long K) {
  SyrkPlan p;
  long steps = (K + 3) / 4;
  if (steps < 1) steps = 1;
  long max_sg = steps / 64;
  if (max_sg < 1) max_sg = 1;
  {
    const long one_round = 1024 / ntiles > 1 ? 1024 / ntiles : 1;
    if (max_sg < one_round) {
      long nst = SYRK_NBUF;
      while ((steps + nst - 1) / nst > one_round) nst += SYRK_NBUF;
      p.SG = (int)((steps + nst - 1) / nst);
      p.nsteps = (int)nst;
      p.Kpad = (int)(p.SG * nst * 4);
      p.nblocks = (long)p.SG * ntiles;
      return p;
    }
  }
  long base = (4096 + ntiles - 1) / ntiles, sg = base;
  double best = -1.0;
  for (long c = (base > 6 ? base - 6 : 1); c <= base + 6; c++) {
    const double per_xcd = (double)ntiles * c / 8.0;
    const double rounds = (double)(long)((per_xcd + 127.0) / 128.0);
    const double eff = per_xcd / (rounds * 128.0);
    if (eff > best + 1e-9) { best = eff; sg = c; }
  }
  if (sg > max_sg) sg = max_sg;
  if (steps / sg < 128 && sg > 1) {
    long one_round = 1024 / ntiles;
    if (one_round < 1) one_round = 1;
    if (one_round < sg) sg = one_round;
  }
  long nst = (steps + sg - 1) / sg;
  nst = (nst + SYRK_NBUF - 1) / SYRK_NBUF * SYRK_NBUF;
  p.SG = (int)sg;
  p.nsteps = (int)nst;
  p.Kpad = (int)(sg * nst * 4);
  p.nblocks = sg * ntiles;
  return p;
}

void launch_syrk_sparse(hipStream_t s, const double *Gt, int npad, const int *jobs, const int *items, const int *chunk_ids,
                        int nsteps, long nitems, double *part) {
  hipLaunchKernelGGL(k_hessian_syrk_sparse, dim3((unsigned)nitems), dim3(64), 0, s, Gt, npad, jobs, items, chunk_ids, nsteps,
                     nitems, part);
}

void launch_syrk(hipStream_t s, const double *Gt, int npad, int ntiles, const int *tileIJ, const SyrkPlan &p,
                 double *part) {
  hipLaunchKernelGGL(k_hessian_syrk, dim3((unsigned)p.nblocks), dim3(64), 0, s, Gt, npad, ntiles, tileIJ,
                     p.nsteps, p.nblocks, part);
}

template <class Sink>
__device__ __forceinline__ void reduce_tiles(const double *__restrict__ part, int SG, long tile_total, Sink sink,
                                             int bid, int nb) {
  for (long t = (long)bid * blockDim.x + threadIdx.x; t < tile_total; t += (long)nb * blockDim.x) {
    double s0 = 0.0, s1 = 0.0, s2 = 0.0, s3 = 0.0;
    const double *pp = part + t;
    int g = 0;
    for (; g + 3 < SG; g += 4) {
      s0 += pp[(size_t)g * tile_total];
      s1 += pp[(size_t)(g + 1) * tile_total];
      s2 += pp[(size_t)(g + 2) * tile_total];
      s3 += pp[(size_t)(g + 3) * tile_total];
    }
    for (; g < SG; g++) s0 += pp[(size_t)g * tile_total];
    sink(t, (s0 + s1) + (s2 + s3));
  }
}

template <class Sink>
__device__ __forceinline__ void reduce_tiles_quads(const double *__restrict__ part, int SG, long tile_total, Sink sink, int bid, int nb) {
  const int c = threadIdx.x & 3;
  const int full = SG / 4;
  for (long t = ((long)bid * blockDim.x + threadIdx.x) >> 2; t < tile_total; t += ((long)nb * blockDim.x) >> 2) {
    const double *pp = part + t + (size_t)c * tile_total;
    double s = 0.0;
    int m = 0;
    for (; m + 3 < full; m += 4) {
      const double v0 = pp[(size_t)(4 * m) * tile_total], v1 = pp[(size_t)(4 * m + 4) * tile_total],
                   v2 = pp[(size_t)(4 * m + 8) * tile_total], v3 = pp[(size_t)(4 * m + 12) * tile_total];
      s += v0;
      s += v1;
      s += v2;
      s += v3;
    }
    for (; m < full; m++) s += pp[(size_t)(4 * m) * tile_total];
    if (c == 0)
      for (int g = 4 * full; g < SG; g++) s += part[(size_t)g * tile_total + t];
    s += __shfl_xor(s, 1, 64);
    s += __shfl_xor(s, 2, 64);
    if (c == 0) sink(t, s);
  }
}

template <class Sink>
__device__ __forceinline__ void reduce_tiles_csr(const double *__restrict__ part, const int *__restrict__ ptr, long tile_total,
                                                 Sink sink, int bid, int nb) {
  for (long t = (long)bid * blockDim.x + threadIdx.x; t < tile_total; t += (long)nb * blockDim.x) {
    const int job = (int)(t / TILE_ELEMS);
    const long e = t - (long)job * TILE_ELEMS;
    const int s0 = ptr[job], s1 = ptr[job + 1];
    double a0 = 0.0, a1 = 0.0, a2 = 0.0, a3 = 0.0;
    int g = s0;
    for (; g + 3 < s1; g += 4) {
      a0 += part[(size_t)g * TILE_ELEMS + e];
      a1 += part[(size_t)(g + 1) * TILE_ELEMS + e];
      a2 += part[(size_t)(g + 2) * TILE_ELEMS + e];
      a3 += part[(size_t)(g + 3) * TILE_ELEMS + e];
    }
    for (; g < s1; g++) a0 += part[(size_t)g * TILE_ELEMS + e];
    sink(t, (a0 + a1) + (a2 + a3));
  }
}

__device__ __forceinline__ void reduce_dacc(const double *__restrict__ dpart, int nblk, int dacc_len, int dacc_cap,
                                            const double *__restrict__ rpart, int nr, double *__restrict__ red_dacc,
                                            double *__restrict__ red_r, int bid) {
  __shared__ double sq[256];
  const int jl = threadIdx.x & 63, q = threadIdx.x >> 6;
  const int j = bid * 64 + jl;
  double s = 0.0;
  if (j < dacc_len) {
    const int chunk = (nblk + 3) / 4;
    const int b0 = q * chunk, b1 = min(nblk, b0 + chunk);
    double a[8];
#pragma unroll
    for (int k = 0; k < 8; k++) a[k] = 0.0;
    int b = b0;
    for (; b + 7 < b1; b += 8) {
#pragma unroll
      for (int k = 0; k < 8; k++) a[k] += dpart[(size_t)(b + k) * dacc_len + j];
    }
    for (; b < b1; b++) a[0] += dpart[(size_t)b * dacc_len + j];
    s = ((a[0] + a[1]) + (a[2] + a[3])) + ((a[4] + a[5]) + (a[6] + a[7]));
  }
  sq[threadIdx.x] = s;
  __syncthreads();
  if (q == 0 && j < dacc_len) red_dacc[j] = (sq[jl] + sq[64 + jl]) + (sq[128 + jl] + sq[192 + jl]);
  if (q == 0 && j >= dacc_len && j < dacc_cap) red_dacc[j] = 0.0;
  if (bid == 0) {
    __syncthreads();
    double r = 0.0;
    for (int t = threadIdx.x; t < nr; t += 256) r += rpart[t];
    sq[threadIdx.x] = r;
    __syncthreads();
    for (int k = 128; k > 0; k >>= 1) {
      if (threadIdx.x < k) sq[threadIdx.x] += sq[threadIdx.x + k];
      __syncthreads();
    }
    if (threadIdx.x == 0) { red_r[0] = sq[0]; red_r[1] = 0.0; }
  }
}

__global__ __launch_bounds__(256) void k_reduce_all(const double *__restrict__ part, int SG, const int *__restrict__ csr_ptr, long tile_total,
                                                    int tile_blocks, const double *__restrict__ dpart, int nblk, int dacc_len, int dacc_cap,
                                                    const double *__restrict__ rpart, int nr, double *__restrict__ red, long dacc_off, long r_off, int quads) {
  if ((int)blockIdx.x < tile_blocks) {
    auto to_payload = [&](long t, double v) { red[t] = v; };
    if (csr_ptr) reduce_tiles_csr(part, csr_ptr, tile_total, to_payload, blockIdx.x, tile_blocks);
    else if (quads) reduce_tiles_quads(part, SG, tile_total, to_payload, blockIdx.x, tile_blocks);
    else reduce_tiles(part, SG, tile_total, to_payload, blockIdx.x, tile_blocks);
  } else {
    reduce_dacc(dpart, nblk, dacc_len, dacc_cap, rpart, nr, red + dacc_off, red + r_off, (int)blockIdx.x - tile_blocks);
  }
}

void launch_reduce(hipStream_t s, const double *part, int SG, long tile_total, const double *dpart, int nblk,
                   int dacc_len, const double *rpart, int nr, double *red, long dacc_off, long r_off, const int *csr_ptr) {
  const int dacc_cap = (int)(r_off - dacc_off);
  static const bool no_quads = getenv("BALM_REDUCE_QUADS") && getenv("BALM_REDUCE_QUADS")[0] == '0';
  const int quads = !csr_ptr && !no_quads && tile_total <= 32768 && SG >= 8;
  int grid = (int)(((quads ? 4 : 1) * tile_total + 255) / 256);
  if (grid > 8192) grid = 8192;
  hipLaunchKernelGGL(k_reduce_all, dim3(grid + (dacc_cap + 63) / 64), dim3(256), 0, s, part, SG, csr_ptr, tile_total, grid, dpart, nblk, dacc_len,
                     dacc_cap, rpart, nr, red, dacc_off, r_off, quads);
}

__device__ __forceinline__ int sym3(int r, int c) {
  if (r > c) { int t = r; r = c; c = t; }
  return r == 0 ? c : (r == 1 ? 2 + c : 5);
}

template <int FORM>
__device__ __forceinline__ double blockdiag_at(const double *__restrict__ dacc, int W, int i, int r, int c) {
  const double *d = dacc + i;
  if (FORM == 0) {
    if (r < 3 && c < 3) return d[(size_t)(6 + sym3(r, c)) * W];
    if (r < 3 && c >= 3) return d[(size_t)(12 + 3 * r + (c - 3)) * W];
    if (r >= 3 && c < 3) return d[(size_t)(12 + 3 * c + (r - 3)) * W];
    return d[(size_t)(21 + sym3(r - 3, c - 3)) * W];
  } else {
    if (r < 3 && c < 3) return d[(size_t)(6 + 3 * r + c) * W];
    if (r < 3 && c >= 3) return d[(size_t)(15 + 3 * r + (c - 3)) * W];
    if (r >= 3 && c < 3) return d[(size_t)(15 + 3 * c + (r - 3)) * W];
    return d[(size_t)(24 + sym3(r - 3, c - 3)) * W];
  }
}

template <int FORM>
__global__ __launch_bounds__(256) void k_assemble(const double *__restrict__ red, long dacc_off,
                                                  const int *__restrict__ tileIJ, int ntiles, int W,
                                                  double *__restrict__ H, double *__restrict__ g, const double *__restrict__ r_in,
                                                  double *__restrict__ r_out) {
  const int n = 6 * W;
  if (r_out && blockIdx.x == 0 && threadIdx.x == 0) *r_out = *r_in;
  const long total = (long)ntiles * TILE_ELEMS;
  const double *dacc = red + dacc_off;
  for (long t = (long)blockIdx.x * blockDim.x + threadIdx.x; t < total; t += (long)gridDim.x * blockDim.x) {
    const int tile = (int)(t / TILE_ELEMS);
    const int e = (int)(t - (long)tile * TILE_ELEMS);
    const int lane = e & 63, slot = e >> 6;
    const int reg = slot & 3, mt = slot >> 2;
    const int rc = tileIJ[tile * 25 + mt];
    const int row = (rc >> 16) * 16 + (lane >> 4) + 4 * reg;
    const int col = (rc & 0xffff) * 16 + (lane & 15);
    if (row >= n || col >= n || row > col) continue;
    double val = -red[t];
    const int pi = row / 6, pj = col / 6;
    if (pi == pj) {
      const int r = row - 6 * pi, c = col - 6 * pi;
      val += blockdiag_at<FORM>(dacc, W, pi, r, c);
      if (FORM == 1 && r != c) {
        H[(size_t)row * n + col] = -red[t] + blockdiag_at<FORM>(dacc, W, pi, c, r);
        H[(size_t)col * n + row] = val;
        continue;
      }
    }
    H[(size_t)col * n + row] = val;
    H[(size_t)row * n + col] = val;
  }
  for (long t = (long)blockIdx.x * blockDim.x + threadIdx.x; t < n; t += (long)gridDim.x * blockDim.x) {
    const int i = (int)(t / 6), k = (int)(t - 6 * (t / 6));
    g[t] = dacc[(size_t)k * W + i];
  }
}

void launch_assemble(hipStream_t s, int form, const double *red, long dacc_off, const int *tileIJ, int ntiles, int W,
                     double *H, double *g, const double *r_in, double *r_out) {
  long total = (long)ntiles * TILE_ELEMS;
  int grid = (int)((total + 255) / 256);
  if (grid > 4096) grid = 4096;
  if (form == 0)
    hipLaunchKernelGGL(k_assemble<0>, dim3(grid), dim3(256), 0, s, red, dacc_off, tileIJ, ntiles, W, H, g, r_in, r_out);
  else
    hipLaunchKernelGGL(k_assemble<1>, dim3(grid), dim3(256), 0, s, red, dacc_off, tileIJ, ntiles, W, H, g, r_in, r_out);
}


}
```

### balm_amd/csrc/kernels_cov.hip

```cpp
#include <cfloat>

#include "balm_internal.h"

namespace balm {

namespace {

typedef double d2 __attribute__((ext_vector_type(2)));

__device__ __forceinline__ void cross3(const double a[3], const double b[3], double o[3]) {
  o[0] = a[1] * b[2] - a[2] * b[1];
  o[1] = a[2] * b[0] - a[0] * b[2];
  o[2] = a[0] * b[1] - a[1] * b[0];
}

__device__ __forceinline__ void g1_top(const double w[4], double g[3][9]) {
#pragma unroll
  for (int r = 0; r < 3; r++)
#pragma unroll
    for (int c = 0; c < 9; c++) g[r][c] = 0.0;
  g[0][0] = w[0]; g[0][1] = w[1]; g[0][2] = w[2]; g[0][6] = w[3];
  g[1][1] = w[0]; g[1][3] = w[1]; g[1][4] = w[2]; g[1][7] = w[3];
  g[2][2] = w[0]; g[2][4] = w[1]; g[2][5] = w[2]; g[2][8] = w[3];
}
// ... 219 lines not shown
            cross3(col, u0, x);
            KM[0][c] = x[0]; KM[1][c] = x[1]; KM[2][c] = x[2];
          }
          double S6[6][6];
#pragma unroll
          for (int r = 0; r < 3; r++) {
            const double row[3] = {KM[r][0], KM[r][1], KM[r][2]};
            double x[3];
            cross3(row, u0, x);
#pragma unroll
            for (int c = 0; c < 3; c++) S6[r][c] = x[c];
          }
          {
            const double m3[3] = {M[0][3], M[1][3], M[2][3]};
            double km3[3];
            cross3(m3, u0, km3);
#pragma unroll
            for (int r = 0; r < 3; r++)
#pragma unroll
              for (int c = 0; c < 3; c++) { S6[r][3 + c] = km3[r] * u0[c]; S6[3 + r][3 + c] = M[3][3] * u0[r] * u0[c]; }
          }
          const double w2 = coe * coe * c2 * c2;
          int t = 0;
#pragma unroll
          for (int r = 0; r < 6; r++)
#pragma unroll
            for (int k = r; k < 6; k++) sacc[(t++) * W + i] += w2 * S6[r][k];
        }
        {
          double m0[3], m1[3], m2[3], cvec[3];
          const double vu1 = vbar[0] * u1[0] + vbar[1] * u1[1] + vbar[2] * u1[2];
          const double vu2 = vbar[0] * u2[0] + vbar[1] * u2[1] + vbar[2] * u2[2];
#pragma unroll
          for (int r = 0; r < 3; r++) {
            cvec[r] = b[r] - N * vbar[r];
            m0[r] = Pw[r][0] * u0[0] + Pw[r][1] * u0[1] + Pw[r][2] * u0[2] - b[r] * vu0;
            m1[r] = Pw[r][0] * u1[0] + Pw[r][1] * u1[1] + Pw[r][2] * u1[2] - b[r] * vu1;
            m2[r] = Pw[r][0] * u2[0] + Pw[r][1] * u2[1] + Pw[r][2] * u2[2] - b[r] * vu2;
          }
          const double s0 = cvec[0] * u0[0] + cvec[1] * u0[1] + cvec[2] * u0[2];
          const double s1 = cvec[0] * u1[0] + cvec[1] * u1[1] + cvec[2] * u1[2];
          const double s2 = cvec[0] * u2[0] + cvec[1] * u2[1] + cvec[2] * u2[2];
          double x01[3], x10[3], x02[3], x20[3], bxu[3];
          cross3(m0, u1, x01); cross3(m1, u0, x10);
          cross3(m0, u2, x02); cross3(m2, u0, x20);
          cross3(b, u0, bxu);
          const double c3 = -2.0 * iNN * iNN;
#pragma unroll
          for (int r = 0; r < 3; r++) {
            at[r][0] = c2 * (x01[r] + x10[r]); at[3 + r][0] = c2 * (s0 * u1[r] + s1 * u0[r]);
            at[r][1] = c2 * (x02[r] + x20[r]); at[3 + r][1] = c2 * (s0 * u2[r] + s2 * u0[r]);
            at[r][2] = c3 * bxu[r];            at[3 + r][2] = c3 * N * u0[r];
          }
        }
      }
      if (!ONEPASS) {
#pragma unroll
        for (int c = 0; c < 3; c++)
#pragma unroll
          for (int r = 0; r < 6; r += 2) {
            *reinterpret_cast<d2 *>(gx + (size_t)c * npad + 6 * i + r) = (d2){at[r][c], at[r + 1][c]};
            *reinterpret_cast<d2 *>(gy + (size_t)c * npad + 6 * i + r) = (d2){rr[r][c], rr[r + 1][c]};
          }
      }
    }
    for (int r = 6 * W + threadIdx.x; r < npad; r += blockDim.x)
#pragma unroll
      for (int c = 0; c < 3; c++) { gx[(size_t)c * npad + r] = 0.0; gy[(size_t)c * npad + r] = 0.0; }

#pragma unroll
    for (int t = 0; t < 6; t++) {
      double s = q[t];
#pragma unroll
      for (int off = 32; off > 0; off >>= 1) s += __shfl_xor(s, off, 64);
      if (lane == 0) sq[wv][t] = s;
    }
    __syncthreads();
    double Q[6];
#pragma unroll
    for (int t = 0; t < 6; t++) {
      double s = sq[0][t];
      for (int w = 1; w < nwv; w++) s += sq[w][t];
      Q[t] = s;
    }
    double C[3][3] = {{0, 0, 0}, {0, 0, 0}, {0, 0, 0}}, Ci[3][3] = {{0, 0, 0}, {0, 0, 0}, {0, 0, 0}};
    {
      const double Qm[3][3] = {{Q[0], Q[1], Q[2]}, {Q[1], Q[3], Q[4]}, {Q[2], Q[4], Q[5]}};
      double d = Qm[0][0];
      if (d > 0) { C[0][0] = sqrt(d); C[1][0] = Qm[1][0] / C[0][0]; C[2][0] = Qm[2][0] / C[0][0]; }
      d = Qm[1][1] - C[1][0] * C[1][0];
      if (Qm[1][1] > 0 && d > 1e-12 * Qm[1][1]) { C[1][1] = sqrt(d); C[2][1] = (Qm[2][1] - C[2][0] * C[1][0]) / C[1][1]; }
      d = Qm[2][2] - C[2][0] * C[2][0] - C[2][1] * C[2][1];
      if (Qm[2][2] > 0 && d > 1e-12 * Qm[2][2]) C[2][2] = sqrt(d);
      const double i0 = C[0][0] > 0 ? 1.0 / C[0][0] : 0.0, i1 = C[1][1] > 0 ? 1.0 / C[1][1] : 0.0,
                   i2 = C[2][2] > 0 ? 1.0 / C[2][2] : 0.0;
      Ci[0][0] = i0; Ci[1][1] = i1; Ci[2][2] = i2;
      Ci[1][0] = -C[1][0] * i0 * i1;
      Ci[2][1] = -C[2][1] * i1 * i2;
      Ci[2][0] = -(C[2][0] * Ci[0][0] + C[2][1] * Ci[1][0]) * i2;
    }
    if (ONEPASS) {
      const int i0 = (int)threadIdx.x - lane;
      if (i0 < W) {
        const int nval = 6 * min(64, W - i0);
        double *stg = sm + (12 + COV_DACC) * W + wv * 384;
#pragma unroll
        for (int c = 0; c < 3; c++) {
          double xc[6], yc[6];
#pragma unroll
          for (int r = 0; r < 6; r++) {
            const double y = rr[r][0] * Ci[c][0] + rr[r][1] * Ci[c][1] + rr[r][2] * Ci[c][2];
            const double x = at[r][0] * C[0][c] + at[r][1] * C[1][c] + at[r][2] * C[2][c];
            xc[r] = coe * (x + y);
            yc[r] = coe * y;
          }
          auto flush = [&](const double col[6], double *gcol) {
            d2 *q2 = reinterpret_cast<d2 *>(stg + 6 * lane);
            q2[0] = (d2){col[0], col[1]}; q2[1] = (d2){col[2], col[3]}; q2[2] = (d2){col[4], col[5]};
            asm volatile("" ::: "memory");
#pragma unroll
            for (int j = 0; j < 3; j++) {
              const int idx = 2 * (64 * j + lane);
              const d2 w = *reinterpret_cast<const d2 *>(stg + idx);
              if (idx < nval) *reinterpret_cast<d2 *>(gcol + idx) = w;
            }
            asm volatile("" ::: "memory");
          };
          flush(xc, gx + (size_t)c * npad + 6 * i0);
          flush(yc, gy + (size_t)c * npad + 6 * i0);
        }
      }
    } else
    for (int i = threadIdx.x; i < W; i += blockDim.x) {
#pragma unroll
      for (int r = 0; r < 6; r++) {
        double A[3], Rw[3];
#pragma unroll
        for (int c = 0; c < 3; c++) { A[c] = gx[(size_t)c * npad + 6 * i + r]; Rw[c] = gy[(size_t)c * npad + 6 * i + r]; }
#pragma unroll
        for (int c = 0; c < 3; c++) {
          const double y = Rw[0] * Ci[c][0] + Rw[1] * Ci[c][1] + Rw[2] * Ci[c][2];
          const double x = A[0] * C[0][c] + A[1] * C[1][c] + A[2] * C[2][c];
          gx[(size_t)c * npad + 6 * i + r] = coe * (x + y);
          gy[(size_t)c * npad + 6 * i + r] = coe * y;
        }
      }
    }
    __syncthreads();
  }
  double *dp = dpart + (size_t)blockIdx.x * COV_DACC * W;
  for (int t = threadIdx.x; t < COV_DACC * W; t += blockDim.x) dp[t] = sacc[t];
}

__global__ __launch_bounds__(256) void k_cov_reduce_tiles(const double *__restrict__ part, int SG, long tile_total,
                                                          double *__restrict__ red) {
  for (long t = (long)blockIdx.x * blockDim.x + threadIdx.x; t < tile_total; t += (long)gridDim.x * blockDim.x) {
    double s = 0.0;
    for (int g = 0; g < SG; g++) s += part[(size_t)g * tile_total + t];
    red[t] = s;
  }
}

__global__ __launch_bounds__(256) void k_cov_reduce_dacc(const double *__restrict__ dpart, int nblk, int len,
                                                         double *__restrict__ out) {
  __shared__ double sq[256];
  const int jl = threadIdx.x & 63, q = threadIdx.x >> 6;
  const int j = blockIdx.x * 64 + jl;
  const int chunk = (nblk + 3) / 4, b0 = q * chunk, b1 = min(nblk, b0 + chunk);
  double a[8] = {0, 0, 0, 0, 0, 0, 0, 0};
  if (j < len) {
    int b = b0;
    for (; b + 8 <= b1; b += 8)
#pragma unroll
      for (int k = 0; k < 8; k++) a[k] += dpart[(size_t)(b + k) * len + j];
    for (; b < b1; b++) a[0] += dpart[(size_t)b * len + j];
  }
  sq[threadIdx.x] = ((a[0] + a[1]) + (a[2] + a[3])) + ((a[4] + a[5]) + (a[6] + a[7]));
  __syncthreads();
  if (q == 0 && j < len) out[j] = (sq[jl] + sq[64 + jl]) + (sq[128 + jl] + sq[192 + jl]);
}

__global__ __launch_bounds__(256) void k_cov_assemble(const double *__restrict__ redx, const double *__restrict__ redy,
                                                      const double *__restrict__ sdiag, const int *__restrict__ tileIJ,
                                                      int ntiles, int W, double *__restrict__ Rout) {
  const int n = 6 * W;
  const long total = (long)ntiles * TILE_ELEMS;
  for (long t = (long)blockIdx.x * blockDim.x + threadIdx.x; t < total; t += (long)gridDim.x * blockDim.x) {
    const int tile = (int)(t / TILE_ELEMS);
    const int e = (int)(t - (long)tile * TILE_ELEMS);
    const int lane = e & 63, slot = e >> 6;
    const int reg = slot & 3, mt = slot >> 2;
    const int rc = tileIJ[tile * 25 + mt];
    const int row = (rc >> 16) * 16 + (lane >> 4) + 4 * reg;
    const int col = (rc & 0xffff) * 16 + (lane & 15);
    if (row >= n || col >= n || row > col) continue;
    double val = redx[t] - redy[t];
    const int pi = row / 6, pj = col / 6;
    if (pi == pj) {
      const int r = row - 6 * pi, c = col - 6 * pi;
      val += sdiag[(size_t)(r * 6 - r * (r - 1) / 2 + (c - r)) * W + pi];
    }
    Rout[(size_t)col * n + row] = val;
    Rout[(size_t)row * n + col] = val;
  }
}

typedef double d4 __attribute__((ext_vector_type(4)));

__global__ __launch_bounds__(256) void k_sym_permute(const double *__restrict__ src, int n, int nA, const int *__restrict__ perm,
                                                     int inverse, double *__restrict__ dst) {
  const long total = (long)nA * nA;
  for (long t = (long)blockIdx.x * blockDim.x + threadIdx.x; t < total; t += (long)gridDim.x * blockDim.x) {
    const int c = (int)(t / nA), r = (int)(t - (long)c * nA);
    const int pr = perm[r], pc = perm[c];
    if (!inverse) dst[t] = (pr < n && pc < n) ? src[(size_t)pc * n + pr] : 0.0;
    else if (pr < n && pc < n) dst[(size_t)pc * n + pr] = src[t];
  }
}

__global__ __launch_bounds__(256) void k_sym_scale(double *__restrict__ T, int nA, const double *__restrict__ dvec) {
  const long total = (long)nA * nA;
  for (long t = (long)blockIdx.x * blockDim.x + threadIdx.x; t < total; t += (long)gridDim.x * blockDim.x) {
    const int c = (int)(t / nA), r = (int)(t - (long)c * nA);
    T[t] *= dvec[r] * dvec[c];
  }
}

constexpr int TG_LD = NB + 1;
__global__ __launch_bounds__(192) void k_tri_gemm(const double *__restrict__ a, long sai, long sak, const double *__restrict__ b,
                                                  long sbk, long sbj, int nA, int tri, double *__restrict__ C) {
  __shared__ double As[NB * TG_LD], Bs[NB * TG_LD];
  const int tid = threadIdx.x, lane = tid & 63, wv = tid >> 6;
  const int l15 = lane & 15, l4 = lane >> 4;
  const int i0 = blockIdx.x * NB, j0 = blockIdx.y * NB;
  int k0 = 0, k1 = nA;
  if (tri == 1) k1 = min(nA, i0 + NB);
  else if (tri == 2) k1 = min(nA, j0 + NB);
  else if (tri == 3) k0 = i0;
  else if (tri == 4) k0 = j0;
  const int f = tid % NB, g0 = tid / NB;
  const bool a_i_fast = sai == 1, b_k_fast = sbk == 1;
  const double *pa = a_i_fast ? a + (size_t)(i0 + f) + (size_t)g0 * sak : a + (size_t)(i0 + g0) * sai + (size_t)f;
  const long sa_m = a_i_fast ? 4 * sak : 4 * sai, sa_k = a_i_fast ? sak : 1;
  const double *pb = b_k_fast ? b + (size_t)f + (size_t)(j0 + g0) * sbj : b + (size_t)g0 * sbk + (size_t)(j0 + f);
  const long sb_m = b_k_fast ? 4 * sbj : 4 * sbk, sb_k = b_k_fast ? 1 : sbk;
  const int la = a_i_fast ? g0 * TG_LD + f : f * TG_LD + g0, la_m = a_i_fast ? 4 * TG_LD : 4;
  const int lb = b_k_fast ? f * TG_LD + g0 : g0 * TG_LD + f, lb_m = b_k_fast ? 4 : 4 * TG_LD;
  d4 acc[3];
#pragma unroll
  for (int y = 0; y < 3; y++) acc[y] = (d4){0.0, 0.0, 0.0, 0.0};
  double ra[12], rb[12];
  if (k0 < k1) {
#pragma unroll
    for (int m = 0; m < 12; m++) { ra[m] = pa[(size_t)k0 * sa_k + m * sa_m]; rb[m] = pb[(size_t)k0 * sb_k + m * sb_m]; }
  }
  for (int kb = k0; kb < k1; kb += NB) {
    __syncthreads();
#pragma unroll
    for (int m = 0; m < 12; m++) { As[la + m * la_m] = ra[m]; Bs[lb + m * lb_m] = rb[m]; }
    __syncthreads();
    if (kb + NB < k1) {
#pragma unroll
      for (int m = 0; m < 12; m++) { ra[m] = pa[(size_t)(kb + NB) * sa_k + m * sa_m]; rb[m] = pb[(size_t)(kb + NB) * sb_k + m * sb_m]; }
    }
#pragma unroll
    for (int u = 0; u < 12; u++) {
      const double av = As[(4 * u + l4) * TG_LD + 16 * wv + l15];
#pragma unroll
      for (int y = 0; y < 3; y++)
        acc[y] = __builtin_amdgcn_mfma_f64_16x16x4f64(av, Bs[(4 * u + l4) * TG_LD + 16 * y + l15], acc[y], 0, 0, 0);
    }
  }
#pragma unroll
  for (int y = 0; y < 3; y++)
#pragma unroll
    for (int e = 0; e < 4; e++)
      C[(size_t)(j0 + 16 * y + l15) * nA + i0 + 16 * wv + l4 + 4 * e] = acc[y][e];
}

inline int grid1(long total, int bs, int cap) {
  long g = (total + bs - 1) / bs;
  return (int)(g > cap ? cap : (g < 1 ? 1 : g));
}

}

static bool cov_onepass(int W) {
  const char *e = getenv("BALM_COV_ONEPASS");
  return W <= 256 && !(e && e[0] == '0');
}
constexpr size_t COV_STAGE_BYTES = 4 * 384 * sizeof(double);

int cov_factors_grid(int W, int F) {
  size_t lds = (size_t)(12 + COV_DACC) * W * sizeof(double) + (cov_onepass(W) ? COV_STAGE_BYTES : 0);
  int per_cu = (int)(150 * 1024 / lds);
  if (per_cu < 1) per_cu = 1;
  if (per_cu > 4) per_cu = 4;
  int grid = 256 * per_cu;
  if (grid > F) grid = F;
  return grid < 1 ? 1 : grid;
}

hipError_t prepare_device_cov() {
  hipError_t e = hipFuncSetAttribute((const void *)k_cov_factors<true, false>, hipFuncAttributeMaxDynamicSharedMemorySize, 160 * 1024 - 1024);
  if (e == hipSuccess) e = hipFuncSetAttribute((const void *)k_cov_factors<false, false>, hipFuncAttributeMaxDynamicSharedMemorySize, 160 * 1024 - 1024);
  if (e == hipSuccess) e = hipFuncSetAttribute((const void *)k_cov_factors<true, true>, hipFuncAttributeMaxDynamicSharedMemorySize, 160 * 1024 - 1024);
  if (e == hipSuccess) e = hipFuncSetAttribute((const void *)k_cov_factors<false, true>, hipFuncAttributeMaxDynamicSharedMemorySize, 160 * 1024 - 1024);
  return e;
}

void launch_cov_factors(hipStream_t s, const double *cl, const double *ccov, double sigma2, const double *poses,
                        const double *feat, int W, int npad, int F, double *Gx, double *Gy, double *dpart, int nblk) {
  const bool one = cov_onepass(W);
  size_t lds = (size_t)(12 + COV_DACC) * W * sizeof(double) + (one ? COV_STAGE_BYTES : 0);
  int bs = W <= 64 ? 64 : (W <= 128 ? 128 : 256);
#define BALM_COV_FACTORS(E, O) hipLaunchKernelGGL((k_cov_factors<E, O>), dim3(nblk), dim3(bs), lds, s, cl, ccov, sigma2, poses, feat, W, npad, F, Gx, Gy, dpart)
  if (ccov) { if (one) BALM_COV_FACTORS(true, true); else BALM_COV_FACTORS(true, false); }
  else { if (one) BALM_COV_FACTORS(false, true); else BALM_COV_FACTORS(false, false); }
#undef BALM_COV_FACTORS
}

void launch_cov_reduce_tiles(hipStream_t s, const double *part, int SG, long tile_total, double *red) {
  hipLaunchKernelGGL(k_cov_reduce_tiles, dim3(grid1(tile_total, 256, 8192)), dim3(256), 0, s, part, SG, tile_total, red);
}

void launch_cov_reduce_dacc(hipStream_t s, const double *dpart, int nblk, int W, double *out) {
  hipLaunchKernelGGL(k_cov_reduce_dacc, dim3((COV_DACC * W + 63) / 64), dim3(256), 0, s, dpart, nblk, COV_DACC * W, out);
}

void launch_cov_assemble(hipStream_t s, const double *redx, const double *redy, const double *sdiag, const int *tileIJ,
                         int ntiles, int W, double *Rout) {
  hipLaunchKernelGGL(k_cov_assemble, dim3(grid1((long)ntiles * TILE_ELEMS, 256, 4096)), dim3(256), 0, s, redx, redy, sdiag,
                     tileIJ, ntiles, W, Rout);
}

void launch_congruence_inverse(balm_ctx *c, const double *Rraw, double *T0, double *T1, double *Rcov) {
  hipStream_t s = c->stream;
  const int n = c->n, nA = c->nA;
  const long ldA = 2L * nA + NB;
  const double *M = c->d_A + (size_t)(nA + NB);
  const dim3 grid(nA / NB, nA / NB), blk(192);
  const int g1 = grid1((long)nA * nA, 256, 4096);
  hipLaunchKernelGGL(k_sym_permute, dim3(g1), dim3(256), 0, s, Rraw, n, nA, c->d_perm, 0, T0);
  hipLaunchKernelGGL(k_tri_gemm, grid, blk, 0, s, M, ldA, 1L, T0, 1L, (long)nA, nA, 1, T1);
  hipLaunchKernelGGL(k_tri_gemm, grid, blk, 0, s, T1, 1L, (long)nA, M, 1L, ldA, nA, 2, T0);
  hipLaunchKernelGGL(k_sym_scale, dim3(g1), dim3(256), 0, s, T0, nA, c->d_dvec);
  hipLaunchKernelGGL(k_tri_gemm, grid, blk, 0, s, M, 1L, ldA, T0, 1L, (long)nA, nA, 3, T1);
  hipLaunchKernelGGL(k_tri_gemm, grid, blk, 0, s, T1, 1L, (long)nA, M, ldA, 1L, nA, 4, T0);
  hipLaunchKernelGGL(k_sym_permute, dim3(g1), dim3(256), 0, s, T0, n, nA, c->d_perm, 1, Rcov);
}

}
```

### include/balm_hip.h

```cpp
#ifndef BALM_HIP_H
#define BALM_HIP_H

#include <stddef.h>

#ifdef __cplusplus
extern "C" {
#endif

typedef struct balm_ctx balm_ctx;

enum { BALM_FORM_LEFT = 0, BALM_FORM_RIGHT = 1 };

enum {
  BALM_OK = 0,
  BALM_ERR_ARG = 1,
  BALM_ERR_HIP = 2,
  BALM_ERR_STATE = 3,
  BALM_ERR_TOO_FEW_PLANES = 4,
  BALM_ERR_NUMERIC = 5
};

enum {
  BALM_FLAG_TIMING = 1,
  BALM_FLAG_LOOPBACK_SHARDS = 2,
  BALM_FLAG_SYRK_INT8 = 4
};

typedef struct balm_iter_log {
  double r1, r2, u, v, q, q1;
  int accepted;
  int hess_evaluated;
} balm_iter_log;

typedef struct balm_lm_opts {
  int form;
  double u0;
  int max_iter;
  double rel_tol;
  int min_planes_per_pose;
  int force_hess;
  int no_stop;
  int verbose;
  int reanchor;
  double abs_tol;
} balm_lm_opts;

balm_ctx *balm_create(int win_size, int device, int flags);
void balm_destroy(balm_ctx *ctx);

int balm_prewarm(int device);

balm_ctx *balm_create_multi(int win_size, int first_device, int n_devices, int flags);

int balm_comm_unique_id(void *id128);
int balm_comm_init_rank(balm_ctx *ctx, int n_ranks, int rank, const void *id128);
int balm_comm_info(balm_ctx *ctx, long *out4);

int balm_set_features(balm_ctx *ctx, int F, const double *clusters, const double *fix,
                      const double *coeffs);

typedef void (*balm_fill_clusters_fn)(void *user, int f0, int f1, double *dst);
int balm_set_features_cb(balm_ctx *ctx, int F, balm_fill_clusters_fn fill, void *user, const double *fix,
                         const double *coeffs);

int balm_evaluate(balm_ctx *ctx, int form, const double *poses, int head, int end, double *Hess,
                  double *JacT, double *residual);

int balm_only_residual(balm_ctx *ctx, const double *poses, double *residual);

int balm_solve_damped(balm_ctx *ctx, const double *Hess, const double *JacT, double u, double *dxi,
                      double *q1);

int balm_damping_iter(balm_ctx *ctx, const balm_lm_opts *opts, double *poses_inout,
                      balm_iter_log *log, int *n_iters);

int balm_build_clusters(balm_ctx *ctx, int F, const float *xyz, const int *feat_id,
                        const int *pose_id, long n_pts, const double *fix, const double *coeffs,
                        double *clusters_out);

int balm_build_clusters_planes(balm_ctx *ctx, int F, const void *const *plane_points, const long *plane_count,
                               size_t stride_bytes, size_t pose_offset_bytes, const double *fix, const double *coeffs,
                               double *clusters_out);

typedef struct balm_voxel_opts {
  double voxel_size;
  float eigen_thr[3];
  int min_ps;
  int layer_limit;
  int min_observers;
  int fix_frames;
  double max_plane_dist;
  double max_lambda21;
  double max_lambda0;
  int want_point_features;
  int fix_point_limit;
  int defer_recut;
} balm_voxel_opts;
void balm_voxel_defaults(balm_voxel_opts *opts);
int balm_associate(balm_ctx *ctx, const balm_voxel_opts *opts, const float *xyz, const int *frame_id,
                   long n_pts, const double *poses, int *F_out, long *n_root_voxels);

int balm_associate_scans(balm_ctx *ctx, const balm_voxel_opts *opts, int n_scans, const void *const *scan_points,
                         const long *scan_count, size_t stride_bytes, const double *poses, int *F_out,
                         long *n_root_voxels);

int balm_window_open(balm_ctx *ctx, const balm_voxel_opts *opts);
int balm_window_recut(balm_ctx *ctx);
int balm_window_add_scan(balm_ctx *ctx, const float *xyz, long n_pts, const double *pose12);
int balm_window_add_scan_strided(balm_ctx *ctx, const void *points, long n_pts, size_t stride_bytes, const double *pose12);
int balm_window_features(balm_ctx *ctx, int *F_out);
int balm_window_marginalize(balm_ctx *ctx, int mg_size, const double *poses);
int balm_window_info(balm_ctx *ctx, int *scans_in_window, long *points, long *nodes);
int balm_window_get_points(balm_ctx *ctx, float *xyz, int *slot, int *feature, long capacity, long *n_out);
int balm_window_close(balm_ctx *ctx);

int balm_get_features(balm_ctx *ctx, double *clusters, double *coeffs, int *layer);

int balm_get_association(balm_ctx *ctx, double *fix, int *point_feature);

int balm_pose_covariance(balm_ctx *ctx, const double *poses, const double *cluster_cov, double point_sigma,
                         double *Rcov, double *Rcov_raw);

typedef int (*balm_allreduce_fn)(void *dev_buf, long n_doubles, void *user);
int balm_set_allreduce(balm_ctx *ctx, balm_allreduce_fn fn, void *user);

enum {
  BALM_T_MOMENTS = 0,
  BALM_T_FACTORS = 1,
  BALM_T_SYRK = 2,
  BALM_T_ASSEMBLE = 3,
  BALM_T_SOLVE = 4,
  BALM_T_UPDATE = 5,
  BALM_T_BUILD = 6,
  BALM_T_VOXEL = 7,
  BALM_T_COV = 8,
  BALM_T_COMM = 9,
  BALM_T_UPLOAD = 10,
  BALM_T_COUNT = 11
};
int balm_get_timing(balm_ctx *ctx, double *ms, long *count);
int balm_get_shard_timing(balm_ctx *ctx, int shard, double *ms, long *count);

int balm_get_solve_trace(balm_ctx *ctx, long long *ticks, long capacity, int *dims3);
int balm_reset_timing(balm_ctx *ctx);

int balm_chain_macro_plan(int panels, int helpers, int *table, long capacity);

int balm_work_model(balm_ctx *ctx, double *out4);

const char *balm_last_error(balm_ctx *ctx);
const char *balm_version(void);

#define BALM_ABI_VERSION 6
int balm_abi_version(void);

#ifdef __cplusplus
}
#endif
#endif
```

Before: 248.3.

## Add load-balanced SYRK work-item plan with tile-major partial slots

Introduces an optional balanced SYRK schedule that splits each tile's K range into variable-length items spread over a fixed set of 1024 workgroups. CSR offsets let the reduce kernels sum a variable number of partials per tile. The partial-buffer layout changes to tile-major slots in all paths. The dense plan is cached per context instead of being recomputed every call. Balanced mode is enabled only through an environment variable, and it adds indirection and host-side planning.

```diff
diff --git a/balm_amd/capi.py b/balm_amd/capi.py
--- a/balm_amd/capi.py
+++ b/balm_amd/capi.py
@@ -19,7 +19,7 @@
            "balm_solve_damped", "balm_damping_iter", "balm_build_clusters", "balm_build_clusters_planes", "balm_voxel_defaults", "balm_associate", "balm_associate_scans", "balm_get_features", "balm_get_association", "balm_pose_covariance",
            "balm_window_open", "balm_window_add_scan", "balm_window_add_scan_strided", "balm_window_recut", "balm_window_get_points", "balm_window_features", "balm_window_marginalize", "balm_window_info", "balm_window_close",
            "balm_set_allreduce", "balm_comm_unique_id", "balm_comm_init_rank", "balm_comm_info",
-           "balm_get_timing", "balm_get_shard_timing", "balm_get_solve_trace", "balm_chain_macro_plan", "balm_reset_timing", "balm_work_model", "balm_last_error", "balm_version", "balm_abi_version"]
+           "balm_get_timing", "balm_get_shard_timing", "balm_get_solve_trace", "balm_chain_macro_plan", "balm_syrk_plan", "balm_reset_timing", "balm_work_model", "balm_last_error", "balm_version", "balm_abi_version"]
 
 
 class IterLog(C.Structure):
@@ -110,6 +110,7 @@
         L.balm_get_shard_timing.argtypes = [C.c_void_p, C.c_int, C.c_void_p, C.c_void_p]
         L.balm_get_solve_trace.argtypes = [C.c_void_p, C.c_void_p, C.c_long, C.c_void_p]
         L.balm_chain_macro_plan.argtypes = [C.c_int, C.c_int, C.c_void_p, C.c_long]
+        L.balm_syrk_plan.argtypes = [C.c_int, C.c_long, C.c_int, C.c_void_p, C.c_void_p, C.c_long]
         L.balm_reset_timing.argtypes = [C.c_void_p]
         L.balm_work_model.argtypes = [C.c_void_p, C.c_void_p]
         L.balm_last_error.restype = C.c_char_p
@@ -126,6 +127,21 @@
         raise BalmError(rc, "balm_chain_macro_plan(%d, %d)" % (panels, helpers))
     tab = tab.reshape(helpers, 64)
     return [[(int(e) & 0xffff, int(e) >> 16) for e in row if e >= 0] for row in tab]
+
+
+def syrk_plan(jobs, K, uniform=False):
+    info = np.zeros(4, np.int32)
+    rc = lib().balm_syrk_plan(int(jobs), int(K), int(bool(uniform)), info.ctypes.data_as(C.c_void_p), None, 0)
+    if rc != OK:
+        raise BalmError(rc, "balm_syrk_plan(%d, %d)" % (jobs, K))
+    nwg, nitems = int(info[2]), int(info[3])
+    tab = np.empty(nwg + 1 + 4 * nitems + jobs + 1, np.int32)
+    rc = lib().balm_syrk_plan(int(jobs), int(K), int(bool(uniform)), info.ctypes.data_as(C.c_void_p), tab.ctypes.data_as(C.c_void_p), tab.size)
+    if rc != OK:
+        raise BalmError(rc, "balm_syrk_plan(%d, %d)" % (jobs, K))
+    ptr, items, csr = tab[:nwg + 1], tab[nwg + 1:nwg + 1 + 4 * nitems].reshape(-1, 4), tab[nwg + 1 + 4 * nitems:]
+    return {"balanced": bool(info[0]), "Kpad": int(info[1]), "csr": [int(v) for v in csr],
+            "workgroups": [[tuple(int(v) for v in items[i]) for i in range(int(ptr[b]), int(ptr[b + 1]))] for b in range(nwg)]}
 
 
 def _p(a):
diff --git a/balm_amd/csrc/balm_capi.hip b/balm_amd/csrc/balm_capi.hip
--- a/balm_amd/csrc/balm_capi.hip
+++ b/balm_amd/csrc/balm_capi.hip
@@ -248,11 +248,15 @@
   return K >= 12288L && ctx->W >= 96;
 }
 
+static SyrkPlan dense_plan(const balm_ctx *ctx, int nf) {
+  return nf == ctx->plan_F ? ctx->dplan : plan_syrk(ctx->ntiles, 3L * nf);
+}
+
 int prepare_evaluate(balm_ctx *ctx, int form, int nf) {
   if (nf <= 0) return BALM_OK;
-  const SyrkPlan plan = plan_syrk(ctx->ntiles, 3L * nf);
+  const SyrkPlan plan = dense_plan(ctx, nf);
   int rc;
-  size_t gcols = (size_t)plan.Kpad + 64, parts = (size_t)plan.SG * ctx->ntiles;
+  size_t gcols = (size_t)plan.Kpad + 64, parts = (size_t)plan.nslots;
   if (ctx->sparse && nf == ctx->F) {
     gcols = (size_t)ctx->sp_nchunks * ctx->sp_nsteps * 4 + 64;
     parts = (size_t)ctx->sp_nitems;
@@ -293,7 +297,7 @@
                     ctx->d_red + red_r_off(ctx), ctx->d_scal + slot);
     return BALM_OK;
   }
-  SyrkPlan plan = plan_syrk(ctx->ntiles, 3L * nf);
+  SyrkPlan plan = dense_plan(ctx, nf);
   if ((rc = prepare_evaluate(ctx, form, nf))) return rc;
   const int nblk = factors_grid(W, nf, form);
   hipStream_t s = ctx->stream;
@@ -330,12 +334,13 @@
                          ctx->rowmax_cur_valid ? ctx->d_rowmax : nullptr)) { ctx->err = "INT8 SYRK: unsupported size"; return BALM_ERR_ARG; }
       plan.SG = 1;
     }
-    else launch_syrk(s, ctx->d_Gt, ctx->npad, ctx->ntiles, ctx->d_jobs, plan, ctx->d_part);
+    else launch_syrk(s, ctx->d_Gt, ctx->npad, ctx->ntiles, ctx->d_jobs, plan, ctx->d_plan_wg, ctx->d_plan_items, ctx->d_part);
   }
   {
     Span sp(ctx, BALM_T_ASSEMBLE);
     launch_reduce(s, ctx->d_part, plan.SG, (long)ctx->ntiles * TILE_ELEMS, ctx->d_dpart, nblk, dacc * W,
-                  ctx->d_rpart, nr, ctx->d_red, red_dacc_off(ctx), red_r_off(ctx), sparse ? ctx->d_csr : nullptr);
+                  ctx->d_rpart, nr, ctx->d_red, red_dacc_off(ctx), red_r_off(ctx),
+                  sparse ? ctx->d_csr : (plan.balanced && !int8 ? ctx->d_plan_csr : nullptr));
   }
   if ((rc = hook_allreduce(ctx, ctx->d_red, (long)ctx->red_len))) return rc;
   {
@@ -349,7 +354,7 @@
 int trial_device(balm_ctx *ctx, int form, const double *d_poses, int slot) {
   const int W = ctx->W, F = ctx->F;
   hipStream_t s = ctx->stream;
-  const SyrkPlan plan = plan_syrk(ctx->ntiles, 3L * F);
+  const SyrkPlan plan = dense_plan(ctx, F);
   const bool sparse = ctx->sparse;
   const size_t kpad = sparse ? (size_t)ctx->sp_nchunks * ctx->sp_nsteps * 4 : (size_t)plan.Kpad;
   const int nblk = factors_grid(W, F, form);
@@ -455,6 +460,7 @@
   ctx->device = device;
   ctx->flags = flags;
   ctx->timer.on = (flags & BALM_FLAG_TIMING) != 0;
+  if (const char *pl = getenv("BALM_SYRK")) ctx->syrk_balanced = !strcmp(pl, "balanced");
   auto fail = [&]() -> balm_ctx * { one_destroy(ctx); return nullptr; };
   std::vector<int> jobs, sub;
   {
@@ -533,7 +539,7 @@
   if (ctx->window) { window_close(ctx->window); ctx->window = nullptr; }
   void *ptrs[] = {ctx->d_cl, ctx->d_fix, ctx->d_coe, ctx->d_poses, ctx->d_poses_tmp, ctx->d_C, ctx->d_feat,
                   ctx->d_Gt, ctx->d_Gt2, ctx->d_dpart2, ctx->d_part, ctx->d_dpart, ctx->d_rpart, ctx->d_feat_tmp, ctx->d_rpart_tmp, ctx->d_red, ctx->d_jobs, ctx->d_sub, ctx->d_H,
-                  ctx->d_g, ctx->d_A, ctx->d_Wp, ctx->d_dvec, ctx->d_z, ctx->d_x, ctx->d_perm, ctx->d_dx, ctx->d_scal, ctx->d_arena, ctx->d_pre, ctx->d_flags, ctx->d_minv, ctx->d_macro_tab, ctx->d_trace, ctx->d_slot, ctx->d_items, ctx->d_csr, ctx->d_chunk_ids, ctx->d_stage, ctx->d_i8, ctx->d_rowmax, ctx->d_rowmax2, ctx->d_rowmax_part};
+                  ctx->d_g, ctx->d_A, ctx->d_Wp, ctx->d_dvec, ctx->d_z, ctx->d_x, ctx->d_perm, ctx->d_dx, ctx->d_scal, ctx->d_arena, ctx->d_pre, ctx->d_flags, ctx->d_minv, ctx->d_macro_tab, ctx->d_trace, ctx->d_slot, ctx->d_items, ctx->d_csr, ctx->d_chunk_ids, ctx->d_plan_wg, ctx->d_plan_items, ctx->d_plan_csr, ctx->d_stage, ctx->d_i8, ctx->d_rowmax, ctx->d_rowmax2, ctx->d_rowmax_part};
   for (void *p : ptrs) if (p) hipFree(p);
   if (ctx->h_scal) hipHostFree(ctx->h_scal);
   ctx->ring.release();
@@ -545,8 +551,26 @@
   delete ctx;
 }
 
+static int build_dense_plan(balm_ctx *ctx, int F) {
+  ctx->plan_F = F;
+  ctx->dplan = plan_syrk(ctx->ntiles, 3L * F);
+  if (!ctx->syrk_balanced || syrk_int8_for(ctx, 3L * F)) return BALM_OK;
+  SyrkItems it;
+  if (!plan_syrk_balanced(ctx->ntiles, 3L * F, it)) return BALM_OK;
+  int rc;
+  if ((rc = keep(ctx, &ctx->d_plan_wg, &ctx->cap_plan_wg, it.wg_ptr.size())) || (rc = keep(ctx, &ctx->d_plan_items, &ctx->cap_plan_items, it.items.size())) ||
+      (rc = keep(ctx, &ctx->d_plan_csr, &ctx->cap_plan_csr, it.csr.size())))
+    return rc;
+  HIP_TRY(hipMemcpy(ctx->d_plan_wg, it.wg_ptr.data(), it.wg_ptr.size() * sizeof(int), hipMemcpyHostToDevice));
+  HIP_TRY(hipMemcpy(ctx->d_plan_items, it.items.data(), it.items.size() * sizeof(int), hipMemcpyHostToDevice));
+  HIP_TRY(hipMemcpy(ctx->d_plan_csr, it.csr.data(), it.csr.size() * sizeof(int), hipMemcpyHostToDevice));
+  ctx->dplan = it.p;
+  return BALM_OK;
+}
+
 static int build_sparse_plan(balm_ctx *ctx, int F, const unsigned char *obs) {
   ctx->sparse = false;
+  if (int rc = build_dense_plan(ctx, F)) return rc;
   const char *mode = getenv("BALM_SYRK");
   if (mode && !strcmp(mode, "dense")) return BALM_OK;
   if (syrk_int8_for(ctx, 3L * F)) return BALM_OK;
@@ -1104,11 +1128,11 @@
   int rc = evaluate_device(ctx, BALM_FORM_LEFT, ctx->d_poses, 0, F, 0);
   ctx->feat_cur_valid = false; ctx->gt_cur_valid = false;
   if (rc) return rc;
-  const SyrkPlan plan = plan_syrk(ctx->ntiles, 3L * (F > 0 ? F : 1));
+  const SyrkPlan plan = dense_plan(ctx, F > 0 ? F : 1);
   const size_t gcols = (size_t)plan.Kpad + 64, tiles = (size_t)ctx->ntiles * TILE_ELEMS;
   if ((rc = ensure(ctx, &ctx->d_Gt, &ctx->cap_Gt, 2 * gcols * ctx->npad))) return rc;
   ctx->gt_dirty_cols = ~(size_t)0;
-  if ((rc = ensure(ctx, &ctx->d_part, &ctx->cap_part, (size_t)plan.SG * tiles))) return rc;
+  if ((rc = ensure(ctx, &ctx->d_part, &ctx->cap_part, (size_t)plan.nslots * TILE_ELEMS))) return rc;
   const int nblk = cov_factors_grid(W, F > 0 ? F : 1);
   if ((rc = ensure(ctx, &ctx->d_dpart, &ctx->cap_dpart, (size_t)nblk * DACC_MAX * W))) return rc;
   const bool int8 = F > 0 && syrk_int8_for(ctx, 3L * F);
@@ -1140,14 +1164,15 @@
     e = hipGetLastError();
     if (int8) {
       if (launch_syrk_i8(s, Gx, ctx->npad, ctx->n, 3L * F, ctx->d_sub, ctx->ntiles, ctx->d_i8, ctx->d_part)) e = hipErrorInvalidValue;
-      launch_cov_reduce_tiles(s, ctx->d_part, 1, (long)tiles, redx);
+      launch_cov_reduce_tiles(s, ctx->d_part, 1, nullptr, (long)tiles, redx);
       if (launch_syrk_i8(s, Gy, ctx->npad, ctx->n, 3L * F, ctx->d_sub, ctx->ntiles, ctx->d_i8, ctx->d_part)) e = hipErrorInvalidValue;
-      launch_cov_reduce_tiles(s, ctx->d_part, 1, (long)tiles, redy);
+      launch_cov_reduce_tiles(s, ctx->d_part, 1, nullptr, (long)tiles, redy);
     } else {
-      launch_syrk(s, Gx, ctx->npad, ctx->ntiles, ctx->d_jobs, plan, ctx->d_part);
-      launch_cov_reduce_tiles(s, ctx->d_part, plan.SG, (long)tiles, redx);
-      launch_syrk(s, Gy, ctx->npad, ctx->ntiles, ctx->d_jobs, plan, ctx->d_part);
-      launch_cov_reduce_tiles(s, ctx->d_part, plan.SG, (long)tiles, redy);
+      const int *csr = plan.balanced ? ctx->d_plan_csr : nullptr;
+      launch_syrk(s, Gx, ctx->npad, ctx->ntiles, ctx->d_jobs, plan, ctx->d_plan_wg, ctx->d_plan_items, ctx->d_part);
+      launch_cov_reduce_tiles(s, ctx->d_part, plan.SG, csr, (long)tiles, redx);
+      launch_syrk(s, Gy, ctx->npad, ctx->ntiles, ctx->d_jobs, plan, ctx->d_plan_wg, ctx->d_plan_items, ctx->d_part);
+      launch_cov_reduce_tiles(s, ctx->d_part, plan.SG, csr, (long)tiles, redy);
     }
     launch_cov_reduce_dacc(s, ctx->d_dpart, nblk, W, sdiag);
   }
@@ -1836,6 +1861,19 @@
   return BALM_OK;
 }
 
+int balm_syrk_plan(int jobs, long K, int uniform, int *info4, int *table, long capacity) {
+  if (!info4 || jobs < 1 || K < 1 || K > (1L << 30)) return BALM_ERR_ARG;
+  balm::SyrkItems it;
+  balm::plan_syrk_items(jobs, K, uniform != 0, it);
+  info4[0] = it.p.balanced ? 1 : 0; info4[1] = it.p.Kpad; info4[2] = (int)it.p.nblocks; info4[3] = (int)it.p.nslots;
+  const size_t need = it.wg_ptr.size() + it.items.size() + it.csr.size();
+  if (!table) return BALM_OK;
+  if (capacity < (long)need) return BALM_ERR_ARG;
+  int *q = table;
+  for (const std::vector<int> *v : {&it.wg_ptr, &it.items, &it.csr}) { memcpy(q, v->data(), v->size() * sizeof(int)); q += v->size(); }
+  return BALM_OK;
+}
+
 int balm_reset_timing(balm_ctx *ctx) {
   if (!ctx) return BALM_ERR_ARG;
   for (int k = 0; k < BALM_T_COUNT; k++) { ctx->timer.ms[k] = 0; ctx->timer.cnt[k] = 0; }
@@ -1856,7 +1894,7 @@
   }
   (void)W;
   out4[2] = 216.0 * out4[1];
-  SyrkPlan p = plan_syrk(ctx->ntiles, 3L * (long)F);
+  SyrkPlan p = ctx->multi ? plan_syrk(ctx->ntiles, 3L * (long)F) : dense_plan(ctx, (int)F);
   out4[3] = (double)ctx->ntiles * 25.0 * 2048.0 * ((double)p.Kpad / 4.0);
   if (ctx->sparse && !ctx->multi) out4[3] = ctx->sp_steps * 25.0 * 2048.0;
   if (ctx->multi) {
@@ -1865,7 +1903,7 @@
       const balm_ctx *q = ctx->multi->sub[k];
       if (q->F < 1) continue;
       if (q->sparse) issued += q->sp_steps * 25.0 * 2048.0;
-      else { const SyrkPlan pk = plan_syrk(q->ntiles, 3L * q->F); issued += (double)q->ntiles * 25.0 * 2048.0 * ((double)pk.Kpad / 4.0); }
+      else { const SyrkPlan pk = dense_plan(q, q->F); issued += (double)q->ntiles * 25.0 * 2048.0 * ((double)pk.Kpad / 4.0); }
     }
     out4[3] = issued;
   }
diff --git a/balm_amd/csrc/balm_internal.h b/balm_amd/csrc/balm_internal.h
--- a/balm_amd/csrc/balm_internal.h
+++ b/balm_amd/csrc/balm_internal.h
@@ -38,6 +38,8 @@
   double ms[BALM_T_COUNT] = {0};
   long cnt[BALM_T_COUNT] = {0};
 };
+
+struct SyrkPlan { int SG; int nsteps; int Kpad; long nblocks; long nslots; bool balanced; };
 
 }
 
@@ -94,6 +96,11 @@
   int *d_chunk_ids = nullptr;
   double sp_steps = 0;
   int *d_csr = nullptr;
+  bool syrk_balanced = false;
+  int plan_F = 0;
+  balm::SyrkPlan dplan = {};
+  int *d_plan_wg = nullptr, *d_plan_items = nullptr, *d_plan_csr = nullptr;
+  size_t cap_plan_wg = 0, cap_plan_items = 0, cap_plan_csr = 0;
   int *d_jobs = nullptr;
   int *d_sub = nullptr;
   double *d_H = nullptr;
@@ -182,10 +189,12 @@
 int launch_moments_factors(hipStream_t s, int form, const double *cl, const double *poses, const double *fix, const double *coe, int W,
                            int npad, int F, double *Gt, double *dpart, int nblk, const int *slot, double *feat, double *rpart,
                            unsigned long long *rowmax = nullptr, double *rowmax_part = nullptr);
-struct SyrkPlan { int SG; int nsteps; int Kpad; long nblocks; };
 SyrkPlan plan_syrk(int ntiles, long K);
+struct SyrkItems { SyrkPlan p; std::vector<int> wg_ptr, items, csr; };
+bool plan_syrk_balanced(int ntiles, long K, SyrkItems &out);
+void plan_syrk_items(int ntiles, long K, bool uniform, SyrkItems &out);
 void launch_syrk(hipStream_t s, const double *Gt, int npad, int ntiles, const int *tileIJ, const SyrkPlan &p,
-                 double *part);
+                 const int *wg_ptr, const int *items, double *part);
 void launch_syrk_sparse(hipStream_t s, const double *Gt, int npad, const int *jobs, const int *items, const int *chunk_ids,
                         int nsteps, long nitems, double *part);
 void launch_reduce(hipStream_t s, const double *part, int SG, long tile_elems_total, const double *dpart, int nblk,
@@ -286,7 +295,7 @@
 int cov_factors_grid(int W, int F);
 void launch_cov_factors(hipStream_t s, const double *cl, const double *ccov, double sigma2, const double *poses,
                         const double *feat, int W, int npad, int F, double *Gx, double *Gy, double *dpart, int nblk);
-void launch_cov_reduce_tiles(hipStream_t s, const double *part, int SG, long tile_total, double *red);
+void launch_cov_reduce_tiles(hipStream_t s, const double *part, int SG, const int *csr, long tile_total, double *red);
 void launch_cov_reduce_dacc(hipStream_t s, const double *dpart, int nblk, int W, double *out);
 void launch_cov_assemble(hipStream_t s, const double *redx, const double *redy, const double *sdiag, const int *tileIJ,
                          int ntiles, int W, double *Rout);
diff --git a/balm_amd/csrc/kernels_accum.hip b/balm_amd/csrc/kernels_accum.hip
--- a/balm_amd/csrc/kernels_accum.hip
+++ b/balm_amd/csrc/kernels_accum.hip
@@ -919,13 +919,22 @@
 
 __global__ __launch_bounds__(64) void k_hessian_syrk(const double *__restrict__ Gt, int npad, int njobs,
                                                      const int *__restrict__ jobs, int nsteps, long nblocks,
+                                                     const int *__restrict__ wg_ptr, const int *__restrict__ items,
                                                      double *__restrict__ part) {
-  const long bid = xcd_remap(blockIdx.x, nblocks);
-  const int tile = (int)(bid % njobs);
-  const int sg = (int)(bid / njobs);
-  BALM_SYRK_ZERO_ACC();
-  syrk_accumulate(Gt, npad, jobs[4 * tile], jobs[4 * tile + 1], jobs[4 * tile + 2], (size_t)sg * nsteps * 4, nsteps);
-  syrk_write_out(part + ((size_t)sg * njobs + tile) * TILE_ELEMS);
+  int it = (int)blockIdx.x, end = it + 1;
+  if (wg_ptr) { it = wg_ptr[blockIdx.x]; end = wg_ptr[blockIdx.x + 1]; }
+  for (; it < end; it++) {
+    int tile, k0, ns, slot;
+    if (wg_ptr) { tile = items[4 * it]; k0 = items[4 * it + 1]; ns = items[4 * it + 2]; slot = items[4 * it + 3]; }
+    else {
+      const long bid = xcd_remap(it, nblocks);
+      const int sg = (int)(bid / njobs);
+      tile = (int)(bid % njobs); k0 = sg * nsteps; ns = nsteps; slot = tile * (int)(nblocks / njobs) + sg;
+    }
+    BALM_SYRK_ZERO_ACC();
+    syrk_accumulate(Gt, npad, jobs[4 * tile], jobs[4 * tile + 1], jobs[4 * tile + 2], (size_t)k0 * 4, ns);
+    syrk_write_out(part + (size_t)slot * TILE_ELEMS);
+  }
 }
 
 __global__ __launch_bounds__(64) void k_hessian_syrk_sparse(const double *__restrict__ Gt, int npad,
@@ -956,6 +965,7 @@
       p.nsteps = (int)nst;
       p.Kpad = (int)(p.SG * nst * 4);
       p.nblocks = (long)p.SG * ntiles;
+      p.nslots = p.nblocks; p.balanced = false;
       return p;
     }
   }
@@ -979,7 +989,92 @@
   p.nsteps = (int)nst;
   p.Kpad = (int)(sg * nst * 4);
   p.nblocks = sg * ntiles;
+  p.nslots = p.nblocks; p.balanced = false;
   return p;
+}
+
+constexpr int SYRK_ITEM_COST = 8;
+
+bool plan_syrk_balanced(int ntiles, long K, SyrkItems &out) {
+  const SyrkPlan u = plan_syrk(ntiles, K);
+  out.p = u; out.wg_ptr.clear(); out.items.clear(); out.csr.clear();
+  const long steps = (K + 3) / 4, turns = (steps + SYRK_NBUF - 1) / SYRK_NBUF;
+  const int nhelp = 128 - ntiles;
+  if (ntiles < 64 || nhelp < 1 || steps < 16384) return false;
+  const long item_cost = SYRK_ITEM_COST;
+  struct Piece { int job, k0, ns; };
+  std::vector<std::vector<Piece>> wg(1024);
+  long worst = 0;
+  for (int g = 0; g < 8; g++) {
+    const long t0 = turns * g / 8, L = turns * (g + 1) / 8 - t0;
+    long best_m = L, best_cost = L * SYRK_NBUF + item_cost;
+    auto helper_cost = [&](long r) {
+      long hc = 0;
+      const long N = (long)ntiles * r;
+      for (int h = 0; h < nhelp; h++) {
+        const long lo = N * h / nhelp, hi = N * (h + 1) / nhelp;
+        if (hi > lo) hc = std::max(hc, (hi - lo) * SYRK_NBUF + item_cost * ((hi - 1) / r - lo / r + 1));
+      }
+      return hc;
+    };
+    for (long m = L - 1; m >= 1; m--) {
+      const long hc = helper_cost(L - m), c = std::max(m * SYRK_NBUF + item_cost, hc);
+      if (c < best_cost) { best_cost = c; best_m = m; }
+      if (hc > m * SYRK_NBUF + item_cost) break;
+    }
+    worst = std::max(worst, best_cost);
+    const long m = best_m, r = L - m, N = (long)ntiles * r;
+    for (int j = 0; j < ntiles; j++) wg[(size_t)(8 * j + g)].push_back({j, (int)(t0 * SYRK_NBUF), (int)(m * SYRK_NBUF)});
+    for (int h = 0; h < nhelp && r > 0; h++) {
+      const long lo = N * h / nhelp, hi = N * (h + 1) / nhelp;
+      for (long q = lo; q < hi;) {
+        const long j = q / r, e = std::min(hi, (j + 1) * r);
+        wg[(size_t)(8 * (ntiles + h) + g)].push_back({(int)j, (int)((t0 + m + (q - j * r)) * SYRK_NBUF), (int)((e - q) * SYRK_NBUF)});
+        q = e;
+      }
+    }
+  }
+  const long uniform_cost = (u.nblocks + 1023) / 1024 * (u.nsteps + item_cost);
+  if (!(worst * 100 < uniform_cost * 99)) return false;
+  std::vector<std::array<int, 3>> order;
+  out.wg_ptr.assign(1025, 0);
+  for (int b = 0; b < 1024; b++) {
+    for (const Piece &pc : wg[(size_t)b]) {
+      order.push_back({pc.job, pc.k0, (int)(out.items.size() / 4)});
+      out.items.insert(out.items.end(), {pc.job, pc.k0, pc.ns, 0});
+    }
+    out.wg_ptr[(size_t)b + 1] = (int)(out.items.size() / 4);
+  }
+  std::sort(order.begin(), order.end());
+  out.csr.assign((size_t)ntiles + 1, 0);
+  for (size_t k = 0; k < order.size(); k++) {
+    out.items[(size_t)4 * order[k][2] + 3] = (int)k;
+    out.csr[(size_t)order[k][0] + 1] = (int)k + 1;
+  }
+  out.p.SG = 0; out.p.nsteps = 0;
+  out.p.Kpad = (int)(turns * SYRK_NBUF * 4);
+  out.p.nblocks = 1024;
+  out.p.nslots = (long)order.size();
+  out.p.balanced = true;
+  return true;
+}
+
+void plan_syrk_items(int ntiles, long K, bool uniform, SyrkItems &out) {
+  if (!uniform && plan_syrk_balanced(ntiles, K, out)) return;
+  const SyrkPlan &p = out.p = plan_syrk(ntiles, K);
+  out.wg_ptr.resize((size_t)p.nblocks + 1);
+  out.items.resize((size_t)p.nblocks * 4);
+  out.csr.resize((size_t)ntiles + 1);
+  const long q = p.nblocks >> 3, r = p.nblocks & 7;
+  for (long b = 0; b < p.nblocks; b++) {
+    const long x = b & 7, bid = x * q + (x < r ? x : r) + (b >> 3);
+    const int tile = (int)(bid % ntiles), sg = (int)(bid / ntiles);
+    const int item[4] = {tile, sg * p.nsteps, p.nsteps, tile * p.SG + sg};
+    std::copy(item, item + 4, out.items.begin() + 4 * b);
+    out.wg_ptr[(size_t)b] = (int)b;
+  }
+  out.wg_ptr[(size_t)p.nblocks] = (int)p.nblocks;
+  for (int j = 0; j <= ntiles; j++) out.csr[(size_t)j] = j * p.SG;
 }
 
 void launch_syrk_sparse(hipStream_t s, const double *Gt, int npad, const int *jobs, const int *items, const int *chunk_ids,
@@ -989,27 +1084,9 @@
 }
 
 void launch_syrk(hipStream_t s, const double *Gt, int npad, int ntiles, const int *tileIJ, const SyrkPlan &p,
-                 double *part) {
+                 const int *wg_ptr, const int *items, double *part) {
   hipLaunchKernelGGL(k_hessian_syrk, dim3((unsigned)p.nblocks), dim3(64), 0, s, Gt, npad, ntiles, tileIJ,
-                     p.nsteps, p.nblocks, part);
-}
-
-template <class Sink>
-__device__ __forceinline__ void reduce_tiles(const double *__restrict__ part, int SG, long tile_total, Sink sink,
-                                             int bid, int nb) {
-  for (long t = (long)bid * blockDim.x + threadIdx.x; t < tile_total; t += (long)nb * blockDim.x) {
-    double s0 = 0.0, s1 = 0.0, s2 = 0.0, s3 = 0.0;
-    const double *pp = part + t;
-    int g = 0;
-    for (; g + 3 < SG; g += 4) {
-      s0 += pp[(size_t)g * tile_total];
-      s1 += pp[(size_t)(g + 1) * tile_total];
-      s2 += pp[(size_t)(g + 2) * tile_total];
-      s3 += pp[(size_t)(g + 3) * tile_total];
-    }
-    for (; g < SG; g++) s0 += pp[(size_t)g * tile_total];
-    sink(t, (s0 + s1) + (s2 + s3));
-  }
+                     p.nsteps, p.nblocks, p.balanced ? wg_ptr : nullptr, items, part);
 }
 
 template <class Sink>
@@ -1017,20 +1094,21 @@
   const int c = threadIdx.x & 3;
   const int full = SG / 4;
   for (long t = ((long)bid * blockDim.x + threadIdx.x) >> 2; t < tile_total; t += ((long)nb * blockDim.x) >> 2) {
-    const double *pp = part + t + (size_t)c * tile_total;
+    const long job = t / TILE_ELEMS;
+    const double *p0 = part + ((size_t)job * SG) * TILE_ELEMS + (t - job * TILE_ELEMS), *pp = p0 + (size_t)c * TILE_ELEMS;
     double s = 0.0;
     int m = 0;
     for (; m + 3 < full; m += 4) {
-      const double v0 = pp[(size_t)(4 * m) * tile_total], v1 = pp[(size_t)(4 * m + 4) * tile_total],
-                   v2 = pp[(size_t)(4 * m + 8) * tile_total], v3 = pp[(size_t)(4 * m + 12) * tile_total];
+      const double v0 = pp[(size_t)(4 * m) * TILE_ELEMS], v1 = pp[(size_t)(4 * m + 4) * TILE_ELEMS],
+                   v2 = pp[(size_t)(4 * m + 8) * TILE_ELEMS], v3 = pp[(size_t)(4 * m + 12) * TILE_ELEMS];
       s += v0;
       s += v1;
       s += v2;
       s += v3;
     }
-    for (; m < full; m++) s += pp[(size_t)(4 * m) * tile_total];
+    for (; m < full; m++) s += pp[(size_t)(4 * m) * TILE_ELEMS];
     if (c == 0)
-      for (int g = 4 * full; g < SG; g++) s += part[(size_t)g * tile_total + t];
+      for (int g = 4 * full; g < SG; g++) s += p0[(size_t)g * TILE_ELEMS];
     s += __shfl_xor(s, 1, 64);
     s += __shfl_xor(s, 2, 64);
     if (c == 0) sink(t, s);
@@ -1038,12 +1116,12 @@
 }
 
 template <class Sink>
-__device__ __forceinline__ void reduce_tiles_csr(const double *__restrict__ part, const int *__restrict__ ptr, long tile_total,
+__device__ __forceinline__ void reduce_tiles_csr(const double *__restrict__ part, const int *__restrict__ ptr, int SG, long tile_total,
                                                  Sink sink, int bid, int nb) {
   for (long t = (long)bid * blockDim.x + threadIdx.x; t < tile_total; t += (long)nb * blockDim.x) {
     const int job = (int)(t / TILE_ELEMS);
     const long e = t - (long)job * TILE_ELEMS;
-    const int s0 = ptr[job], s1 = ptr[job + 1];
+    const int s0 = ptr ? ptr[job] : job * SG, s1 = ptr ? ptr[job + 1] : s0 + SG;
     double a0 = 0.0, a1 = 0.0, a2 = 0.0, a3 = 0.0;
     int g = s0;
     for (; g + 3 < s1; g += 4) {
@@ -1101,9 +1179,8 @@
                                                     const double *__restrict__ rpart, int nr, double *__restrict__ red, long dacc_off, long r_off, int quads) {
   if ((int)blockIdx.x < tile_blocks) {
     auto to_payload = [&](long t, double v) { red[t] = v; };
-    if (csr_ptr) reduce_tiles_csr(part, csr_ptr, tile_total, to_payload, blockIdx.x, tile_blocks);
-    else if (quads) reduce_tiles_quads(part, SG, tile_total, to_payload, blockIdx.x, tile_blocks);
-    else reduce_tiles(part, SG, tile_total, to_payload, blockIdx.x, tile_blocks);
+    if (quads) reduce_tiles_quads(part, SG, tile_total, to_payload, blockIdx.x, tile_blocks);
+    else reduce_tiles_csr(part, csr_ptr, SG, tile_total, to_payload, blockIdx.x, tile_blocks);
   } else {
     reduce_dacc(dpart, nblk, dacc_len, dacc_cap, rpart, nr, red + dacc_off, red + r_off, (int)blockIdx.x - tile_blocks);
   }
diff --git a/balm_amd/csrc/kernels_cov.hip b/balm_amd/csrc/kernels_cov.hip
--- a/balm_amd/csrc/kernels_cov.hip
+++ b/balm_amd/csrc/kernels_cov.hip
@@ -395,11 +395,14 @@
   for (int t = threadIdx.x; t < COV_DACC * W; t += blockDim.x) dp[t] = sacc[t];
 }
 
-__global__ __launch_bounds__(256) void k_cov_reduce_tiles(const double *__restrict__ part, int SG, long tile_total,
-                                                          double *__restrict__ red) {
+__global__ __launch_bounds__(256) void k_cov_reduce_tiles(const double *__restrict__ part, int SG, const int *__restrict__ csr,
+                                                          long tile_total, double *__restrict__ red) {
   for (long t = (long)blockIdx.x * blockDim.x + threadIdx.x; t < tile_total; t += (long)gridDim.x * blockDim.x) {
+    const int job = (int)(t / TILE_ELEMS);
+    const long e = t - (long)job * TILE_ELEMS;
+    const int s0 = csr ? csr[job] : job * SG, s1 = csr ? csr[job + 1] : s0 + SG;
     double s = 0.0;
-    for (int g = 0; g < SG; g++) s += part[(size_t)g * tile_total + t];
+    for (int g = s0; g < s1; g++) s += part[(size_t)g * TILE_ELEMS + e];
     red[t] = s;
   }
 }
@@ -563,8 +566,8 @@
 #undef BALM_COV_FACTORS
 }
 
-void launch_cov_reduce_tiles(hipStream_t s, const double *part, int SG, long tile_total, double *red) {
-  hipLaunchKernelGGL(k_cov_reduce_tiles, dim3(grid1(tile_total, 256, 8192)), dim3(256), 0, s, part, SG, tile_total, red);
+void launch_cov_reduce_tiles(hipStream_t s, const double *part, int SG, const int *csr, long tile_total, double *red) {
+  hipLaunchKernelGGL(k_cov_reduce_tiles, dim3(grid1(tile_total, 256, 8192)), dim3(256), 0, s, part, SG, csr, tile_total, red);
 }
 
 void launch_cov_reduce_dacc(hipStream_t s, const double *dpart, int nblk, int W, double *out) {
diff --git a/include/balm_hip.h b/include/balm_hip.h
--- a/include/balm_hip.h
+++ b/include/balm_hip.h
@@ -146,6 +146,8 @@
 
 int balm_chain_macro_plan(int panels, int helpers, int *table, long capacity);
 
+int balm_syrk_plan(int jobs, long K, int uniform, int *info4, int *table, long capacity);
+
 int balm_work_model(balm_ctx *ctx, double *out4);
 
 const char *balm_last_error(balm_ctx *ctx);
```

Result: no change. 247.6 (-0.3%).
